# Jimmy2027/MoPoE-MIMIC

Hardware: AMD Instinct MI355X
Metric: samples/sec (higher is better)
Workload: dtype f32

## Files before the change

### include/mopoe_hip.h

```cpp
#ifndef MOPOE_HIP_H
#define MOPOE_HIP_H

#include <stddef.h>
#include <stdint.h>

#ifdef __cplusplus
extern "C" {
#endif

#define MOPOE_ABI_VERSION 20

#define MOPOE_OK 0
#define MOPOE_ERR_ARG (-1)
#define MOPOE_ERR_LAUNCH (-2)
#define MOPOE_ERR_DEVICE (-3)

int mopoe_abi_version(void);
const char* mopoe_last_error(void);

typedef struct {
  int32_t N;
  int32_t Hs, Ws;
  int32_t Hb, Wb;
  int32_t Cin, Cout;
  int32_t kh, kw;
  int32_t sh, sw;
  int32_t ph, pw;
  int32_t transposed;
} mopoe_conv_geom;

typedef struct {
  const double* sums;
  const float* gamma;
  const float* beta;
  const float* rmean;
  const float* rvar;
  double inv_count;
  float eps;
  int32_t C;
  int32_t mode;
} mopoe_bn_ref;

typedef struct {
  const float* mask;
  int32_t kind;
  int32_t rows_per_sample;
} mopoe_mask_ref;

size_t mopoe_conv_workspace_bytes(void);

typedef struct {
  int32_t tile;
  int32_t split;
} mopoe_conv_plan;

int mopoe_conv_fwd(const float* x, const float* wp, const float* bias, float* y,
                   const mopoe_conv_geom* g, const mopoe_bn_ref* bn_in, const mopoe_mask_ref* mask,
                   double* out_stats, const mopoe_conv_plan* plan, void* workspace, size_t workspace_bytes,
                   void* stream);

typedef struct {
  const void* s;
  mopoe_bn_ref bn;
  float a, b;
} mopoe_mix_ref;
int mopoe_conv_fwd_mix(const float* x, const float* wp, const float* bias, float* y, const mopoe_conv_geom* g,
                       const mopoe_bn_ref* bn_in, const mopoe_mask_ref* mask, const mopoe_mix_ref* mix,
                       double* out_stats, const mopoe_conv_plan* plan, void* workspace, size_t workspace_bytes,
                       void* stream);

int mopoe_conv_dgrad(const float* dy, const float* wp, float* dx, const mopoe_conv_geom* g,
                     const mopoe_bn_ref* relu_bn, const float* xin, double* bwd_sums,
                     const mopoe_conv_plan* plan, void* workspace, size_t workspace_bytes, void* stream);

int mopoe_conv_wgrad(const float* x, const float* dy, float* dwp, const mopoe_conv_geom* g,
                     const mopoe_bn_ref* bn_in, int32_t dwp_is_zero, const mopoe_conv_plan* plan, void* stream);

int mopoe_block_out_fwd(const float* s, const float* m, float* out, int64_t rows, int32_t C,
                        const mopoe_bn_ref* bn_s, float a, float b, double* out_stats, void* stream);

int mopoe_bn_relu_apply(const float* x, float* out, int64_t rows, int32_t C, const mopoe_bn_ref* bn, void* stream);

int mopoe_bn_bwd_reduce(const float* g, const float* s, int64_t rows, int32_t C,
                        const mopoe_bn_ref* bn_s, double* sums, void* stream);

int mopoe_block_out_bwd(const float* g, const float* s, float* dm, float* ds, int64_t rows, int32_t C,
                        const mopoe_bn_ref* bn_s, const double* sums, const mopoe_mask_ref* mask,
                        float a, float b, float* dgamma, float* dbeta, float* colsum_dm,
                        float* colsum_ds, void* stream);

int mopoe_bn_bwd_apply(const float* dy, const float* x, const float* add, float* dx, int64_t rows,
                       int32_t C, const mopoe_bn_ref* bn, const double* sums,
                       const mopoe_mask_ref* mask, float* dgamma, float* dbeta, float* colsum_dx,
                       const float* next_s, const mopoe_bn_ref* next_bn, double* next_sums, void* stream);

typedef struct {
  const double* sums;
  float* rmean;
  float* rvar;
  int32_t C;
  int32_t count;
} mopoe_bn_running_desc;
int mopoe_bn_running_update(const mopoe_bn_running_desc* desc, int32_t n, float momentum, void* stream);

int mopoe_colsum(const float* x, float* out, int64_t rows, int32_t C, int32_t out_is_zero, void* stream);

int mopoe_latent_fwd(const float* const mu_in[3], const float* const lv_in[3], const float* eps,
                     int32_t B, int32_t D, const int32_t* row_start, const float* w, float norm,
                     float* mus, float* lvs, float* joint_mu, float* joint_lv, float* z, float* klds,
                     float* joint_div, double* kl_ws, void* stream);

int mopoe_latent_bwd(const float* const mu_in[3], const float* const lv_in[3], const float* eps,
                     int32_t B, int32_t D, const int32_t* row_start, const float* w, float norm,
                     const float* g_mus, const float* g_lvs, const float* g_joint_mu,
                     const float* g_joint_lv, const float* g_z, const float* g_klds,
                     const float* g_joint_div, float* const d_mu_in[3], float* const d_lv_in[3],
                     void* stream);

#define MOPOE_LATENT_MOE 0
#define MOPOE_LATENT_JSD 1
int mopoe_latent_mixture_fwd(int32_t method, const float* const mu_in[3], const float* const lv_in[3],
                             const float* eps, int32_t B, int32_t D, const int32_t* member_row_start,
                             const int32_t* comp_row_start, const float* w, float norm, float* sub_mu,
                             float* sub_lv, float* comp_mu, float* comp_lv, float* joint_mu, float* joint_lv,
                             float* z, float* klds, float* individual_divs, float* joint_div, float* pd_mu,
                             float* pd_lv, double* ws, void* stream);

int mopoe_latent_mixture_bwd(int32_t method, const float* const mu_in[3], const float* const lv_in[3],
                             const float* eps, int32_t B, int32_t D, const int32_t* member_row_start,
                             const int32_t* comp_row_start, const float* w, float norm, const float* g_sub_mu,
                             const float* g_sub_lv, const float* g_comp_mu, const float* g_comp_lv,
                             const float* g_joint_mu, const float* g_joint_lv, const float* g_z,
                             const float* g_klds, const float* g_individual_divs, const float* g_joint_div,
                             const float* g_pd_mu, const float* g_pd_lv, float* const d_mu_in[3],
                             float* const d_lv_in[3], void* stream);

// ... 13 lines not shown
int mopoe_dense_nll_fwd(const float* logp, const float* target, int64_t n, float norm, float* out, double* ws,
                        void* stream);
int mopoe_dense_nll_bwd(const float* target, const float* g, int64_t n, float norm, float* dlogp, void* stream);

int mopoe_laplace_logprob_rows(const float* x_hat, const float* x, int64_t rows, int64_t per_row,
                               int64_t target_rows, float scale, float* out, void* stream);
int mopoe_token_logprob_rows(const float* logp, const float* ids, int64_t rows, int32_t L, int32_t V,
                             int64_t target_rows, float* out, void* stream);
int mopoe_token_softmax_grad(const float* logp, const float* ids, const float* g, int64_t rows, int32_t V, float norm,
                             void* dx, int32_t dx_is_bf16, void* stream);
int mopoe_block_front_stats_bf16(const uint16_t* x, const uint16_t* w1, const float* bias, int64_t rows, int32_t C,
                                 const mopoe_bn_ref* bn1, const mopoe_mask_ref* mask1, double* stats_d1, void* stream);
int mopoe_block_front_apply_bf16(const uint16_t* x, const uint16_t* w1, const float* bias, uint16_t* a2, int64_t rows, int32_t C,
                                 const mopoe_bn_ref* bn1, const mopoe_bn_ref* bn2, const mopoe_mask_ref* mask1, void* stream);
int mopoe_block_front_bwd_bf16(const uint16_t* x, const uint16_t* dh2, const uint16_t* w1, const float* bias, uint16_t* dh1,
                               int64_t rows, int32_t C, const mopoe_bn_ref* bn1, const mopoe_bn_ref* bn2,
                               const mopoe_mask_ref* mask1, const double* sums2, double* sums1, float* dw1, float* dbias,
                               float* dgamma2, float* dbeta2, void* stream);
int mopoe_block_front_stats(const float* x, const float* w1, const float* bias, int64_t rows, int32_t C,
                            const mopoe_bn_ref* bn1, const mopoe_mask_ref* mask1, double* stats_d1, void* stream);
int mopoe_block_front_apply(const float* x, const float* w1, const float* bias, float* a2, int64_t rows, int32_t C,
                            const mopoe_bn_ref* bn1, const mopoe_bn_ref* bn2, const mopoe_mask_ref* mask1, void* stream);
int mopoe_block_front_bwd(const float* x, const float* dh2, const float* w1, const float* bias, float* dh1, int64_t rows, int32_t C,
                          const mopoe_bn_ref* bn1, const mopoe_bn_ref* bn2, const mopoe_mask_ref* mask1, const double* sums2,
                          double* sums1, float* dw1, float* dbias, float* dgamma2, float* dbeta2, void* stream);
int mopoe_lse_rows(const void* logits, int32_t is_bf16, int64_t rows, int32_t V, float* lse, void* stream);
int mopoe_token_nll_logits_fwd(const void* logits, int32_t is_bf16, const float* lse, const float* ids, int64_t rows, int32_t V,
                               float norm, float* out, double* ws, void* stream);
int mopoe_token_softmax_grad_logits(const void* logits, int32_t is_bf16, const float* lse, const float* ids, const float* g,
                                    int64_t rows, int32_t V, float norm, void* dx, void* stream);
int mopoe_dense_logprob_rows(const float* logp, const float* target, int64_t rows, int64_t per_row,
                             int64_t target_rows, float* out, void* stream);

int mopoe_embedding_fwd(const float* ids, const float* table, float* out, int64_t rows, int32_t V,
                        int32_t D, void* stream);
int mopoe_embedding_bwd(const float* ids, const float* gout, float* dtable, int64_t rows, int32_t V,
                        int32_t D, int32_t padding_idx, void* stream);


int mopoe_conv_fwd_bf16(const uint16_t* x, const uint16_t* wp, const float* bias, void* y, int32_t y_is_f32,
                        const mopoe_conv_geom* g, const mopoe_bn_ref* bn_in, const mopoe_mask_ref* mask,
                        double* out_stats, const mopoe_conv_plan* plan, void* workspace, size_t workspace_bytes,
                        void* stream);
int mopoe_conv_fwd_mix_bf16(const uint16_t* x, const uint16_t* wp, const float* bias, uint16_t* y,
                            const mopoe_conv_geom* g, const mopoe_bn_ref* bn_in, const mopoe_mask_ref* mask,
                            const mopoe_mix_ref* mix, double* out_stats, const mopoe_conv_plan* plan, void* workspace,
                            size_t workspace_bytes, void* stream);
int mopoe_conv_dgrad_bf16(const uint16_t* dy, const uint16_t* wp, void* dx, int32_t dx_is_f32, const mopoe_conv_geom* g,
                          const mopoe_bn_ref* relu_bn, const uint16_t* xin, double* bwd_sums,
                          const mopoe_conv_plan* plan, void* workspace, size_t workspace_bytes, void* stream);
int mopoe_conv_wgrad_bf16(const uint16_t* x, const uint16_t* dy, float* dwp, const mopoe_conv_geom* g,
                          const mopoe_bn_ref* bn_in, int32_t dwp_is_zero, const mopoe_conv_plan* plan, void* stream);
int mopoe_edge_expand_bf16(const float* scal, const float* w, uint16_t* out, const mopoe_conv_geom* g, int32_t C,
                           double* stats, void* stream);
int mopoe_edge_wgrad_bf16(const uint16_t* vec, const float* scal, float* dw, const mopoe_conv_geom* g, int32_t C,
                          int32_t dw_is_zero, void* stream);
int mopoe_edge_reduce_bf16(const uint16_t* x, const float* w, const float* bias, float* out, const mopoe_conv_geom* g,
                           int32_t C, void* stream);
int mopoe_bn_relu_apply_bf16(const uint16_t* x, uint16_t* out, int64_t rows, int32_t C, const mopoe_bn_ref* bn, void* stream);
int mopoe_block_out_fwd_bf16(const uint16_t* s, const uint16_t* m, uint16_t* out, int64_t rows, int32_t C,
                             const mopoe_bn_ref* bn_s, float a, float b, double* out_stats, void* stream);
int mopoe_bn_bwd_reduce_bf16(const uint16_t* g, const uint16_t* s, int64_t rows, int32_t C, const mopoe_bn_ref* bn_s,
                             double* sums, void* stream);
int mopoe_block_out_bwd_bf16(const uint16_t* g, const uint16_t* s, uint16_t* dm, uint16_t* ds, int64_t rows, int32_t C,
                             const mopoe_bn_ref* bn_s, const double* sums, const mopoe_mask_ref* mask, float a, float b,
                             float* dgamma, float* dbeta, float* colsum_dm, float* colsum_ds, void* stream);
int mopoe_bn_bwd_apply_bf16(const uint16_t* dy, const uint16_t* x, const uint16_t* add, uint16_t* dx, int64_t rows,
                            int32_t C, const mopoe_bn_ref* bn, const double* sums, const mopoe_mask_ref* mask,
                            float* dgamma, float* dbeta, float* colsum_dx, const uint16_t* next_s,
                            const mopoe_bn_ref* next_bn, double* next_sums, void* stream);
int mopoe_colsum_bf16(const uint16_t* x, float* out, int64_t rows, int32_t C, int32_t out_is_zero, void* stream);
int mopoe_logsoftmax_bwd_bf16out(const float* dy, const float* y, uint16_t* dx, int64_t rows, int32_t V, void* stream);
int mopoe_embedding_fwd_bf16(const float* ids, const float* table, uint16_t* out, int64_t rows, int32_t V, int32_t D,
                             void* stream);
int mopoe_embedding_bwd_bf16(const float* ids, const uint16_t* gout, float* dtable, int64_t rows, int32_t V, int32_t D,
                             int32_t padding_idx, void* stream);

typedef struct {
  float* p;
  const float* g;
  float* m;
  float* v;
  uint16_t* p16;
  int64_t n;
} mopoe_adam_seg;
int mopoe_adam_step(const mopoe_adam_seg* segs, int32_t nseg, float* step, const float* lr_dev, double lr, double beta1,
                    double beta2, double eps, float* coef, void* stream);

#define MOPOE_PROF_KINDS 144
int mopoe_prof_enable(int32_t on);
int mopoe_prof_stamp(uint64_t* slot, void* stream);
int mopoe_prof_collect(int64_t* launches, double* total_ms, double* total_flops, double* total_bytes );

#ifdef __cplusplus
}
#endif
#endif
```

### mopoe-mimic_amd/csrc/adam.hip

```cpp
#include "common.hpp"

namespace mopoe {

constexpr int ADAM_SEGS_PER_LAUNCH = 64;
constexpr int ADAM_CHUNK = 4096;
constexpr int ADAM_THREADS = 256;

struct AdamPack {
  mopoe_adam_seg seg[ADAM_SEGS_PER_LAUNCH];
  int chunk_start[ADAM_SEGS_PER_LAUNCH];
};

__global__ void adam_prep_kernel(float* step, const float* lr_dev, double lr_host, double beta1, double beta2, float* coef) {
  if (threadIdx.x != 0 || blockIdx.x != 0) return;
  const float s = step[0] + 1.f;
  step[0] = s;
  const double lr = lr_dev ? (double)lr_dev[0] : lr_host;
  const float bc1 = (float)(1.0 - pow(beta1, (double)s));
  const float bc2s = (float)sqrt(1.0 - pow(beta2, (double)s));
  coef[0] = (float)(lr / (double)bc1);
  coef[1] = bc2s;
}

struct AdamHyper {
  double beta1, beta2, eps;
  float step_size, bc2_sqrt;
};

__device__ __forceinline__ void adam_one(float& p, float g, float& m, float& v, const AdamHyper& h) {
  m = (float)(h.beta1 * (double)m + (1.0 - h.beta1) * (double)g);
  v = (float)(h.beta2 * (double)v + (1.0 - h.beta2) * (double)g * (double)g);
  const float denom = (float)((double)(sqrtf(v) / h.bc2_sqrt) + h.eps);
  p -= h.step_size * m / denom;
}

__global__ __launch_bounds__(ADAM_THREADS) void adam_kernel(const AdamPack pack, int nseg, const float* __restrict__ coef,
                                                            double beta1, double beta2, double eps) {
  const int tid = threadIdx.x, lane = tid & 63;
  const int b = (int)blockIdx.x;
  static_assert(ADAM_SEGS_PER_LAUNCH == 64, "one prefix entry per lane");
  const unsigned long long le = __ballot(pack.chunk_start[lane] <= b);
  const int si = __builtin_amdgcn_readfirstlane(__popcll(le) - 1);
  if (si < 0 || si >= nseg) return;
  const mopoe_adam_seg s = pack.seg[si];
  const long base = (long)(b - pack.chunk_start[si]) * ADAM_CHUNK;
  AdamHyper h;
  h.beta1 = beta1; h.beta2 = beta2; h.eps = eps;
  h.step_size = coef[0]; h.bc2_sqrt = coef[1];

  const bool vec = ((((uintptr_t)s.p | (uintptr_t)s.g | (uintptr_t)s.m | (uintptr_t)s.v) & 15) == 0) &&
                   (s.p16 == nullptr || (((uintptr_t)s.p16) & 7) == 0);
  if (vec) {
    float4 p[4], g[4], m[4], v[4];
    bool ok[4];
#pragma unroll
    for (int i = 0; i < 4; ++i) {
      const long e = base + (long)(i * ADAM_THREADS + tid) * 4;
      ok[i] = e + 3 < s.n;
      if (ok[i]) {
        g[i] = *reinterpret_cast<const float4*>(s.g + e);
        p[i] = *reinterpret_cast<const float4*>(s.p + e);
        m[i] = *reinterpret_cast<const float4*>(s.m + e);
        v[i] = *reinterpret_cast<const float4*>(s.v + e);
      }
    }
#pragma unroll
    for (int i = 0; i < 4; ++i) {
      if (!ok[i]) continue;
      const long e = base + (long)(i * ADAM_THREADS + tid) * 4;
      adam_one(p[i].x, g[i].x, m[i].x, v[i].x, h);
      adam_one(p[i].y, g[i].y, m[i].y, v[i].y, h);
      adam_one(p[i].z, g[i].z, m[i].z, v[i].z, h);
      adam_one(p[i].w, g[i].w, m[i].w, v[i].w, h);
      *reinterpret_cast<float4*>(s.p + e) = p[i];
      *reinterpret_cast<float4*>(s.m + e) = m[i];
      *reinterpret_cast<float4*>(s.v + e) = v[i];
      if (s.p16) {
        uint2 o;
        o.x = pack_bf16(p[i].x, p[i].y);
        o.y = pack_bf16(p[i].z, p[i].w);
        *reinterpret_cast<uint2*>(s.p16 + e) = o;
      }
    }
    const long tail = s.n & ~3L;
    if (tid == 0 && tail >= base && tail < base + ADAM_CHUNK) {
      for (long e = tail; e < s.n; ++e) {
        float pp = s.p[e], mm = s.m[e], vv = s.v[e];
        adam_one(pp, s.g[e], mm, vv, h);
        s.p[e] = pp; s.m[e] = mm; s.v[e] = vv;
        if (s.p16) s.p16[e] = f32_to_bf16(pp);
      }
    }
  } else {
    for (int i = tid; i < ADAM_CHUNK; i += ADAM_THREADS) {
      const long e = base + i;
      if (e >= s.n) break;
      float pp = s.p[e], mm = s.m[e], vv = s.v[e];
      adam_one(pp, s.g[e], mm, vv, h);
      s.p[e] = pp; s.m[e] = mm; s.v[e] = vv;
      if (s.p16) s.p16[e] = f32_to_bf16(pp);
    }
  }
}

}

using namespace mopoe;

extern "C" int mopoe_adam_step(const mopoe_adam_seg* segs, int32_t nseg, float* step, const float* lr_dev, double lr,
                               double beta1, double beta2, double eps, float* coef, void* stream) {
  if ((!segs && nseg != 0) || nseg < 0 || !coef) { set_error("adam_step: bad arguments"); return MOPOE_ERR_ARG; }
  hipStream_t st = (hipStream_t)stream;
  if (step) {
    hipLaunchKernelGGL(adam_prep_kernel, dim3(1), dim3(64), 0, st, step, lr_dev, lr, beta1, beta2, coef);
    if (int rc = check_launch("adam_prep")) return rc;
  }
  int32_t i = 0;
  while (i < nseg) {
    AdamPack pack;
    int n = 0;
    long blocks = 0;
    for (; i < nseg && n < ADAM_SEGS_PER_LAUNCH; ++i) {
      const mopoe_adam_seg& s = segs[i];
      if (!s.g || s.n == 0) continue;
      if (!s.p || !s.m || !s.v || s.n < 0) { set_error("adam_step: record %d is incomplete", (int)i); return MOPOE_ERR_ARG; }
      const long nb = (s.n + ADAM_CHUNK - 1) / ADAM_CHUNK;
      if (nb > 0x7fffffffL) { set_error("adam_step: record %d has more than 2^43 elements", (int)i); return MOPOE_ERR_ARG; }
      if (blocks + nb > 0x7fffffffL) break;
      pack.seg[n] = s;
      pack.chunk_start[n] = (int)blocks;
      blocks += nb;
      ++n;
    }
    for (int k = n; k < ADAM_SEGS_PER_LAUNCH; ++k) { pack.seg[k] = mopoe_adam_seg{}; pack.chunk_start[k] = 0x7fffffff; }
    if (n == 0) continue;
    hipLaunchKernelGGL(adam_kernel, dim3((unsigned)blocks), dim3(ADAM_THREADS), 0, st, pack, n, coef, beta1, beta2, eps);
    if (int rc = check_launch("adam_step")) return rc;
  }
  return MOPOE_OK;
}
```

### mopoe-mimic_amd/csrc/conv_gemm.hip

```cpp
#include "gemm_common.hpp"

namespace mopoe {

constexpr int BK = 16;
#ifndef TILE_N64_REMAINDER
#define TILE_N64_REMAINDER 64
#endif
#ifndef SPLIT_BLOCKS
#define SPLIT_BLOCKS 256
#endif
#ifndef SPLIT_TARGET
#define SPLIT_TARGET 512
#endif
#ifndef GEMM_8WAVES
#define GEMM_8WAVES 1
#endif
#ifndef PERSIST_BLOCKS
#define PERSIST_BLOCKS 2048
#endif
#ifndef GEMM_MIN_WAVES
#define GEMM_MIN_WAVES 3
#endif
#ifndef GEMM_BK_BIG
#define GEMM_BK_BIG 16
#endif
#ifndef GEMM_LDS_PAD
#define GEMM_LDS_PAD 4
#endif
constexpr int LDS_PAD = GEMM_LDS_PAD;

struct GemmArgs {
  const float* X;
  const float* W;
  float* Y;
  const float* bias;
  int N, Hx, Wx, Hy, Wy, Ck, Cn, Cin_w, Cout_w;
  int kh, kw, sh, sw, ph, pw;
  int form, w_nk;
  int Hq, Wq;
  long rows_per_phase;
  int vecA, vecB;
  mopoe_bn_ref bn_in;
  mopoe_mask_ref mask;
  double* out_stats;
  mopoe_bn_ref relu_bn;
  const float* xin;
  double* bwd_sums;
  unsigned x_bytes, w_bytes;
  int nsplit;
  float* partial;
  int* counters;
  long rows_total;
  int mix;
  float mix_a, mix_b;
  int xcd_remap;
};

__device__ __forceinline__ float epi_round(const GemmArgs&, float x) { return x; }
struct EpiXinRaw { float4 lo, hi; };
constexpr bool EPI_PREFETCH_XIN = false;
__device__ __forceinline__ EpiXinRaw epi_xin_ld(const GemmArgs& a, long yrow, int ncol, bool ok_hi) {
  const float* p = a.xin + yrow * a.Cn + ncol;
  EpiXinRaw r;
  r.lo = *reinterpret_cast<const float4*>(p);
  r.hi = ok_hi ? *reinterpret_cast<const float4*>(p + 4) : make_float4(0.f, 0.f, 0.f, 0.f);
  return r;
}
__device__ __forceinline__ void epi_xin_unpack(const EpiXinRaw& r, float (&xi)[8]) {
  xi[0] = r.lo.x; xi[1] = r.lo.y; xi[2] = r.lo.z; xi[3] = r.lo.w; xi[4] = r.hi.x; xi[5] = r.hi.y; xi[6] = r.hi.z; xi[7] = r.hi.w;
}
__device__ __forceinline__ void epi_store8(const GemmArgs& a, long yrow, int ncol, bool ok_hi, const float (&v)[8]) {
  float* dst = a.Y + yrow * a.Cn + ncol;
  *reinterpret_cast<float4*>(dst) = make_float4(v[0], v[1], v[2], v[3]);
  if (ok_hi) *reinterpret_cast<float4*>(dst + 4) = make_float4(v[4], v[5], v[6], v[7]);
}


__device__ __forceinline__ float4 bld4(__amdgpu_buffer_rsrc_t srd, unsigned byte_off) {
  const u32x4 v = __builtin_amdgcn_raw_buffer_load_b128(srd, byte_off, 0, 0);
  return make_float4(__uint_as_float(v.x), __uint_as_float(v.y), __uint_as_float(v.z), __uint_as_float(v.w));
}

__device__ __forceinline__ float4 bld4s(__amdgpu_buffer_rsrc_t srd, unsigned byte_off, unsigned s_off) {
  const u32x4 v = __builtin_amdgcn_raw_buffer_load_b128(srd, byte_off, s_off, 0);
  return make_float4(__uint_as_float(v.x), __uint_as_float(v.y), __uint_as_float(v.z), __uint_as_float(v.w));
}

__device__ __forceinline__ float4 ld4(const float* p, int nvalid, bool vec) {
  float4 v = make_float4(0.f, 0.f, 0.f, 0.f);
  if (nvalid >= 4 && vec) {
    v = *reinterpret_cast<const float4*>(p);
  } else {
    if (nvalid > 0) v.x = p[0];
    if (nvalid > 1) v.y = p[1];
    if (nvalid > 2) v.z = p[2];
    if (nvalid > 3) v.w = p[3];
  }
  return v;
}

template <int BM, int BN, int WGM, int WGN, int GBK, bool VEC, int SPEC = 0>
__global__ __launch_bounds__(64 * WGM * WGN, (WGM * WGN == 4 ? GEMM_MIN_WAVES : ((BM / WGM) * (BN / WGN) > 64 * 32 ? 2 : 4)))
void gather_gemm_kernel(const GemmArgs a) {
  static_assert(SPEC == 0 || VEC, "specialised loops exist for the vector path only");
  constexpr int NT = 64 * WGM * WGN;
  static_assert(WGM * WGN == 4 || WGM * WGN == 8, "4 or 8 waves per block");
  constexpr int WM = BM / WGM, WN = BN / WGN;
  constexpr int TI = WM / 32, TJ = WN / 32;
  constexpr int A_LD = BM + LDS_PAD, B_LD = BN + LDS_PAD;
  constexpr int KQ = GBK / 4;
  constexpr int RPP = NT / KQ;
  constexpr int A_PER_THR = BM / RPP;
  static_assert(BM % RPP == 0, "A tile rows must be a multiple of the rows covered per pass");
  constexpr int B_PER_THR_NK = (BN + RPP - 1) / RPP;
  constexpr int N4 = BN / 4;
  constexpr int B_PER_THR_KN = (GBK * N4 + NT - 1) / NT;
  constexpr int B_PER_THR = B_PER_THR_NK > B_PER_THR_KN ? B_PER_THR_NK : B_PER_THR_KN;

  constexpr int STG_LD = WN + 4;
  constexpr int A_FLOATS = 2 * GBK * A_LD, B_FLOATS = 2 * GBK * B_LD;
  constexpr int STG_FLOATS = VEC ? (NT / 64) * 32 * STG_LD : 0;
  constexpr int SMEM_FLOATS = (A_FLOATS + B_FLOATS) > STG_FLOATS ? (A_FLOATS + B_FLOATS) : STG_FLOATS;
  __shared__ __attribute__((aligned(16))) float smem[SMEM_FLOATS];
  __shared__ __attribute__((aligned(16))) float bnS[MAX_BN_C];
  __shared__ __attribute__((aligned(16))) float bnT[MAX_BN_C];
  __shared__ __attribute__((aligned(16))) float epi[5][VEC ? BN : 4];
  __shared__ int s_ticket;
  float* const As0 = smem;
  float* const Bs0 = smem + A_FLOATS;
#define AS_(buf, k, r) As0[((buf) * GBK + (k)) * A_LD + (r)]
#define BS_(buf, k, r) Bs0[((buf) * GBK + (k)) * B_LD + (r)]

  const int tid = threadIdx.x;
  const int lane = tid & 63, wave = tid >> 6;
  const int wm = wave / WGN, wn = wave % WGN;
  unsigned lbx = blockIdx.x, lby = blockIdx.y, lbz = blockIdx.z;
  if (a.xcd_remap) {
    const unsigned inner = gridDim.y * gridDim.z;
// ... 780 lines not shown
__global__ __launch_bounds__(256) void splitk_epilogue_kernel(const GemmArgs a) {
  __shared__ float cs[2][4][64];
  const int tx = threadIdx.x & 63, ty = threadIdx.x >> 6;
  const int n = blockIdx.x * 64 + tx;
  const bool nok = n < a.Cn;
  const bool do_relu_bn = a.relu_bn.mode != 0;
  const float bias = (nok && a.bias) ? a.bias[n] : 0.f;
  BnC rb = {0.f, 0.f, 0.f, 0.f};
  if (nok && do_relu_bn) rb = bn_coef(a.relu_bn, n);
  const long stride = a.rows_total * (long)a.Cn;
  float s1 = 0.f, s2 = 0.f;
  if (nok) {
    for (long row = (long)blockIdx.y * 4 + ty; row < a.rows_total; row += (long)gridDim.y * 4) {
      const float* p = a.partial + row * a.Cn + n;
      float acc8[8] = {0.f, 0.f, 0.f, 0.f, 0.f, 0.f, 0.f, 0.f};
      int s = 0;
      for (; s + 8 <= a.nsplit; s += 8) {
#pragma unroll
        for (int u = 0; u < 8; ++u) acc8[u] += p[(long)(s + u) * stride];
      }
      for (; s < a.nsplit; ++s) acc8[s & 7] += p[(long)s * stride];
      float x = bias + (((acc8[0] + acc8[1]) + (acc8[2] + acc8[3])) + ((acc8[4] + acc8[5]) + (acc8[6] + acc8[7])));
      if (a.mask.kind != 0) x *= mask_at(a.mask, row, n, a.Cn);
      if (do_relu_bn) {
        const float xi = a.xin[row * a.Cn + n];
        x = (fmaf(xi, rb.scale, rb.shift) > 0.f) ? x : 0.f;
        s1 += x;
        s2 += x * ((xi - rb.mean) * rb.rstd);
      } else {
        s1 += x;
        s2 += x * x;
      }
      a.Y[row * a.Cn + n] = x;
    }
  }
  double* sums = do_relu_bn ? a.bwd_sums : a.out_stats;
  if (sums) {
    cs[0][ty][tx] = s1;
    cs[1][ty][tx] = s2;
    __syncthreads();
    if (ty == 0 && nok) {
      atomic_add_f64(sums + n, (double)((cs[0][0][tx] + cs[0][1][tx]) + (cs[0][2][tx] + cs[0][3][tx])));
      atomic_add_f64(sums + a.Cn + n, (double)((cs[1][0][tx] + cs[1][1][tx]) + (cs[1][2][tx] + cs[1][3][tx])));
    }
  }
}


#include "gemm_glds_common.inc"
#include "conv_gemm_glds.inc"
#include "conv_gemm_glds_parity.inc"


static int launch_gather(const float* X, const float* W, const float* bias, float* Y, const mopoe_conv_geom* g,
                         int dest_on_small, int Ck, int Cn, int w_nk, const mopoe_bn_ref* bn_in,
                         const mopoe_mask_ref* mask, double* out_stats, const mopoe_bn_ref* relu_bn,
                         const float* xin, double* bwd_sums, const mopoe_conv_plan* plan, void* ws, size_t ws_bytes,
                         hipStream_t stream, const mopoe_mix_ref* mix = nullptr) {
  int* counters = nullptr;
  if (ws && ws_bytes > WS_COUNTER_BYTES) { counters = (int*)ws; ws = (char*)ws + WS_COUNTER_BYTES; ws_bytes -= WS_COUNTER_BYTES; }
  else { ws = nullptr; ws_bytes = 0; }
  GemmArgs a;
  a.X = X; a.W = W; a.Y = Y; a.bias = bias;
  a.N = g->N; a.Ck = Ck; a.Cn = Cn; a.Cin_w = g->Cin; a.Cout_w = g->Cout;
  a.kh = g->kh; a.kw = g->kw; a.sh = g->sh; a.sw = g->sw; a.ph = g->ph; a.pw = g->pw;
  a.w_nk = w_nk;
  int nphase;
  if (dest_on_small) {
    a.form = 0; a.Hx = g->Hb; a.Wx = g->Wb; a.Hy = g->Hs; a.Wy = g->Ws; a.Hq = g->Hs; a.Wq = g->Ws; nphase = 1;
  } else {
    a.form = 1; a.Hx = g->Hs; a.Wx = g->Ws; a.Hy = g->Hb; a.Wy = g->Wb; a.Hq = g->Hb / g->sh; a.Wq = g->Wb / g->sw;
    nphase = g->sh * g->sw;
  }
  a.rows_per_phase = (long)g->N * a.Hq * a.Wq;
  a.rows_total = (long)g->N * a.Hy * a.Wy;
  a.vecA = (Ck % 4 == 0) && aligned16(X);
  a.vecB = (g->Cout % 4 == 0) && aligned16(W);
  const size_t xb = (size_t)g->N * a.Hx * a.Wx * Ck * sizeof(float);
  const size_t wb = (size_t)g->kh * g->kw * g->Cin * g->Cout * sizeof(float);
  const bool vec = a.vecA && a.vecB && xb < (1ull << 31) && wb < (1ull << 31) && Cn % 4 == 0 && aligned16(Y) &&
                   (!xin || aligned16(xin)) && (!mask || mask->kind == 0 || aligned16(mask->mask));
  a.x_bytes = (unsigned)std::min<size_t>(xb, 0x7fffffffu);
  a.w_bytes = (unsigned)std::min<size_t>(wb, 0x7fffffffu);
  mopoe_bn_ref none = {};
  mopoe_mask_ref nomask = {nullptr, 0, 1};
  a.bn_in = bn_in ? *bn_in : none;
  a.mask = mask ? *mask : nomask;
  a.out_stats = out_stats;
  a.relu_bn = relu_bn ? *relu_bn : none;
  a.xin = xin; a.bwd_sums = bwd_sums;
  a.mix = 0; a.mix_a = a.mix_b = 0.f;
  static const bool xcd_remap_g = !getenv("MOPOE_NO_XCD_REMAP");
  a.xcd_remap = xcd_remap_g ? 1 : 0;
  if (mix) {
    if (!mix->s || mix->bn.mode == 0 || relu_bn || xin) { set_error("conv_fwd_mix: needs s and its BatchNorm"); return MOPOE_ERR_ARG; }
    if (!vec || !aligned16(mix->s)) { set_error("conv_fwd_mix: channel counts must be multiples of 4 and tensors 16-byte aligned"); return MOPOE_ERR_ARG; }
    a.mix = 1; a.mix_a = mix->a; a.mix_b = mix->b;
    a.relu_bn = mix->bn; a.xin = (const float*)mix->s;
  }
  a.nsplit = 1; a.partial = nullptr; a.counters = nullptr;
  static const bool dbg_nostats = getenv("MOPOE_DEBUG_NOSTATS") != nullptr;
  if (dbg_nostats) { a.out_stats = nullptr; a.bwd_sums = nullptr; }
  if (a.bn_in.mode != 0 && (a.bn_in.C != Ck || Ck > MAX_BN_C)) { set_error("bn_in channel mismatch (%d vs %d)", a.bn_in.C, Ck); return MOPOE_ERR_ARG; }
  if (a.relu_bn.mode != 0 && (a.relu_bn.C != Cn || !a.xin)) { set_error("relu_bn needs xin and C == %d", Cn); return MOPOE_ERR_ARG; }
  if (a.mask.kind != 0 && !a.mask.mask) { set_error("mask pointer missing"); return MOPOE_ERR_ARG; }
  if (a.mask.kind == 1 && a.mask.rows_per_sample != a.Hy * a.Wy) { set_error("channel mask: rows_per_sample must be Hout*Wout"); return MOPOE_ERR_ARG; }
  if (a.rows_total >= (1L << 31) || (long)g->N * a.Hx * a.Wx >= (1L << 31)) { set_error("conv: more than 2^31 rows"); return MOPOE_ERR_ARG; }

  int cfg;
  bool emu = false;
  if (Cn > 64) cfg = (a.rows_per_phase > 64 || Cn >= 256) ? 0 : 2;
  else cfg = a.rows_per_phase >= 256L * 64 ? 1 : 2;
#ifdef TILE_N64_REMAINDER
  if (cfg == 0 && (Cn % 128) == 64 && a.rows_per_phase >= 256L * TILE_N64_REMAINDER) cfg = 1;
#endif
  if (plan && plan->tile >= 0) {
    if (plan->tile > 19) { set_error("conv plan: tile %d (see mopoe_conv_plan in mopoe_hip.h: 0..19)", plan->tile); return MOPOE_ERR_ARG; }
    cfg = plan->tile;
    if (cfg >= 16) {
      if (a.bn_in.mode != 0) { set_error("conv plan: tile %d (split-bf16 products) has no BN-on-load form", cfg); return MOPOE_ERR_ARG; }
      emu = true;
      cfg -= 4;
    }
    if (cfg >= 12 && (!vec || Ck % 32 != 0 || (a.bn_in.mode != 0 && cfg == 13))) {
      set_error("conv plan: tile %d (LDS-DMA family) needs the vector path, K channels %% 32 == 0 (Ck = %d) and, with BN on load, tile 12, 14 or 15", cfg, Ck);
      return MOPOE_ERR_ARG;
    }
    if (cfg >= 3 && !vec) cfg = cfg == 3 ? 0 : 2;
    if ((cfg == 5 || cfg == 6) && Ck % 32 != 0) cfg -= 3;
    if (cfg >= 8 && cfg < 12 && (!vec || Ck % 8 != 0 || a.mix)) cfg = (cfg == 8) ? 0 : (cfg == 9 ? 1 : (cfg == 10 ? 2 : 4));
  }
  static const int TILE_BM[16] = {128, 256, 64, 256, 128, 64, 128, 128, 128, 256, 64, 128, 128, 128, 64, 256};
  static const int TILE_BN[16] = {128, 64, 64, 128, 64, 64, 64, 128, 128, 64, 64, 64, 128, 64, 64, 128};
  const int bm = TILE_BM[cfg], bn = TILE_BN[cfg];
  const long nMt = ceil_div(a.rows_per_phase, bm);
  const int nNt = ceil_div(Cn, bn);
  const int gbk = (cfg == 5 || cfg == 6 || cfg >= 12) ? 32 : (cfg >= 8 ? 8 : 16);
  const int nkc = ceil_div(Ck, gbk);
  const int iters = (dest_on_small ? g->kh * g->kw : std::max(1, (g->kh / g->sh) * (g->kw / g->sw))) * nkc;
  const long blocks = nMt * nNt * nphase;
  const size_t per = (size_t)a.rows_total * Cn * sizeof(float);
  if (plan && plan->split > 0) {
    long ns = std::min<long>(plan->split, iters);
    if (ns >= 2 && (!ws || (size_t)ns * per > ws_bytes)) {
      set_error("conv plan: split %ld needs %zu workspace bytes (have %zu)", ns, (size_t)ns * per, ws ? ws_bytes : (size_t)0);
      return MOPOE_ERR_ARG;
    }
    if (ns >= 2) { a.nsplit = (int)ns; a.partial = (float*)ws; }
  } else if (ws && blocks < SPLIT_BLOCKS && iters * gbk >= 256) {
    long ns = std::min<long>((SPLIT_TARGET + blocks - 1) / blocks, (long)iters * gbk / 128);
    if ((size_t)ns * per > ws_bytes) ns = (long)(ws_bytes / per);
    if (ns >= 2) { a.nsplit = (int)ns; a.partial = (float*)ws; }
  }
  const bool in_kernel_reduce = vec && (cfg < 8 || cfg >= 12);
  if (a.partial && in_kernel_reduce) {
    if (blocks > (long)(WS_COUNTER_BYTES / sizeof(int))) { set_error("conv: split reduction over %ld output tiles (at most %zu)", blocks, WS_COUNTER_BYTES / sizeof(int)); return MOPOE_ERR_ARG; }
    a.counters = counters;
  }
  const long persist = cfg >= 12 ? (cfg == 15 ? 256 : 512)
                                 : (cfg >= 8 ? 4096 : ((cfg == 2 || cfg >= 4) ? PERSIST_BLOCKS * 3 / 2 : PERSIST_BLOCKS));
  long gx = std::min<long>(nMt, std::max<long>(1, persist / ((long)nNt * nphase * a.nsplit)));
  double taps_eff = dest_on_small ? (double)g->kh * g->kw : (double)g->kh * g->kw / ((double)g->sh * g->sw);
  const double flops = 2.0 * (double)g->N * a.Hy * a.Wy * (double)Cn * (double)Ck * taps_eff;
  {
    const int spec = (vec && Ck % gbk == 0) ? (w_nk ? 3 : (a.bn_in.mode != 0 ? 2 : 1)) : 0;
    const double abytes = ((double)g->N * a.Hx * a.Wx * Ck + (double)a.rows_total * Cn) * sizeof(float);
    ProfScope prof(stream, flops, emu ? PROF_F32_GLDS_EMU + (cfg - 12) * 2 + (spec == 3 ? 1 : 0)
                                      : cfg >= 12 ? PROF_F32_GLDS + (cfg - 12) * 3 + (spec - 1)
                                            : (cfg >= 8 ? PROF_DIRECT + (cfg - 8) * 4 + spec
                                                        : (vec ? PROF_GATHER_VEC + cfg * 4 + spec : PROF_GATHER_SCALAR + cfg)), abytes);
    dim3 grid((unsigned)gx, nNt, nphase * a.nsplit);
#define MOPOE_LAUNCH_TILE(BM_, BN_, WM_, WN_, BK_, THREADS_)                                                                    \
  do {                                                                                                                          \
    if (spec == 1) hipLaunchKernelGGL((gather_gemm_kernel<BM_, BN_, WM_, WN_, BK_, true, 1>), grid, dim3(THREADS_), 0, stream, a);      \
    else if (spec == 2) hipLaunchKernelGGL((gather_gemm_kernel<BM_, BN_, WM_, WN_, BK_, true, 2>), grid, dim3(THREADS_), 0, stream, a); \
    else if (spec == 3) hipLaunchKernelGGL((gather_gemm_kernel<BM_, BN_, WM_, WN_, BK_, true, 3>), grid, dim3(THREADS_), 0, stream, a); \
    else hipLaunchKernelGGL((gather_gemm_kernel<BM_, BN_, WM_, WN_, 16, true, 0>), grid, dim3(THREADS_), 0, stream, a);                \
  } while (0)
#define MOPOE_LAUNCH_DIRECT(WM_, WN_, TI_, TJ_)                                                                                   \
  do {                                                                                                                          \
    if (spec == 1) hipLaunchKernelGGL((direct_gemm_kernel<WM_, WN_, TI_, TJ_, 1>), grid, dim3(64 * WM_ * WN_), 0, stream, a);      \
    else if (spec == 2) hipLaunchKernelGGL((direct_gemm_kernel<WM_, WN_, TI_, TJ_, 2>), grid, dim3(64 * WM_ * WN_), 0, stream, a); \
    else hipLaunchKernelGGL((direct_gemm_kernel<WM_, WN_, TI_, TJ_, 3>), grid, dim3(64 * WM_ * WN_), 0, stream, a);                \
  } while (0)
#define MOPOE_LAUNCH_GLDS(BM_, BN_, WM_, WN_, ST_)                                                                                       \
  do {                                                                                                                                \
    if (spec == 1) hipLaunchKernelGGL((gather_gemm_f32_glds_kernel<BM_, BN_, WM_, WN_, 1, ST_>), grid, dim3(64 * WM_ * WN_), 0, stream, a); \
    else hipLaunchKernelGGL((gather_gemm_f32_glds_kernel<BM_, BN_, WM_, WN_, 3, ST_>), grid, dim3(64 * WM_ * WN_), 0, stream, a);          \
  } while (0)
#define MOPOE_LAUNCH_GLDS_EMU(BM_, BN_, WM_, WN_, ST_)                                                                                   \
  do {                                                                                                                                \
    if (spec == 1) hipLaunchKernelGGL((gather_gemm_f32_glds_kernel<BM_, BN_, WM_, WN_, 1, ST_, 1>), grid, dim3(64 * WM_ * WN_), 0, stream, a); \
    else hipLaunchKernelGGL((gather_gemm_f32_glds_kernel<BM_, BN_, WM_, WN_, 3, ST_, 1>), grid, dim3(64 * WM_ * WN_), 0, stream, a);          \
  } while (0)
    if (emu) {
      if (cfg == 12) MOPOE_LAUNCH_GLDS_EMU(128, 128, 2, 2, 2);
      else if (cfg == 13) MOPOE_LAUNCH_GLDS_EMU(128, 64, 2, 2, 3);
      else if (cfg == 14) MOPOE_LAUNCH_GLDS_EMU(64, 64, 2, 2, 4);
      else MOPOE_LAUNCH_GLDS_EMU(256, 128, 4, 2, 3);
    }
#undef MOPOE_LAUNCH_GLDS_EMU
    else if (cfg >= 12) {
      if (spec == 2) {
        if (cfg == 12) hipLaunchKernelGGL((gather_gemm_f32_glds_kernel<128, 128, 2, 2, 2, 2>), grid, dim3(256), 0, stream, a);
        else if (cfg == 14) hipLaunchKernelGGL((gather_gemm_f32_glds_kernel<64, 64, 2, 2, 2, 4>), grid, dim3(256), 0, stream, a);
        else hipLaunchKernelGGL((gather_gemm_f32_glds_kernel<256, 128, 4, 2, 2, 2>), grid, dim3(512), 0, stream, a);
      }
      else if (cfg == 12) MOPOE_LAUNCH_GLDS(128, 128, 2, 2, 2);
      else if (cfg == 13) MOPOE_LAUNCH_GLDS(128, 64, 2, 2, 3);
      else if (cfg == 14) MOPOE_LAUNCH_GLDS(64, 64, 2, 2, 4);
      else MOPOE_LAUNCH_GLDS(256, 128, 4, 2, 2);
    }
#undef MOPOE_LAUNCH_GLDS
    else if (cfg == 8) MOPOE_LAUNCH_DIRECT(2, 2, 2, 2);
    else if (cfg == 9) MOPOE_LAUNCH_DIRECT(4, 1, 2, 2);
    else if (cfg == 10) MOPOE_LAUNCH_DIRECT(2, 2, 1, 1);
    else if (cfg == 11) MOPOE_LAUNCH_DIRECT(2, 1, 2, 2);
    else if (vec) {
      if (cfg == 0) MOPOE_LAUNCH_TILE(128, 128, 2, 4, 16, 512);
      else if (cfg == 1) MOPOE_LAUNCH_TILE(256, 64, 4, 2, 16, 512);
      else if (cfg == 3) MOPOE_LAUNCH_TILE(256, 128, 4, 2, 16, 512);
      else if (cfg == 4) MOPOE_LAUNCH_TILE(128, 64, 2, 2, 16, 256);
      else if (cfg == 5) MOPOE_LAUNCH_TILE(64, 64, 2, 2, 32, 256);
      else if (cfg == 6) MOPOE_LAUNCH_TILE(128, 64, 2, 2, 32, 256);
      else if (cfg == 7) MOPOE_LAUNCH_TILE(128, 128, 2, 2, 16, 256);
      else MOPOE_LAUNCH_TILE(64, 64, 2, 2, 16, 256);
    } else {
      if (cfg == 0) hipLaunchKernelGGL((gather_gemm_kernel<128, 128, 2, 2, GEMM_BK_BIG, false>), grid, dim3(256), 0, stream, a);
      else if (cfg == 1) hipLaunchKernelGGL((gather_gemm_kernel<256, 64, 4, 1, 16, false>), grid, dim3(256), 0, stream, a);
      else hipLaunchKernelGGL((gather_gemm_kernel<64, 64, 2, 2, 16, false>), grid, dim3(256), 0, stream, a);
    }
#undef MOPOE_LAUNCH_TILE
#undef MOPOE_LAUNCH_DIRECT
    if (int rc = check_launch("gather_gemm")) return rc;
    if (a.partial && !in_kernel_reduce) {
      dim3 eg(ceil_div(Cn, 64), std::min<long>(ceil_div(a.rows_total, 4), EPI_MAX_BLOCKS_Y));
      hipLaunchKernelGGL(splitk_epilogue_kernel, eg, dim3(256), 0, stream, a);
      if (int rc = check_launch("splitk_epilogue")) return rc;
    }
  }
  return MOPOE_OK;
}

}

using namespace mopoe;

extern "C" size_t mopoe_conv_workspace_bytes(void) { return WS_RECOMMENDED; }

extern "C" int mopoe_conv_fwd(const float* x, const float* wp, const float* bias, float* y, const mopoe_conv_geom* g,
                              const mopoe_bn_ref* bn_in, const mopoe_mask_ref* mask, double* out_stats,
                              const mopoe_conv_plan* plan, void* workspace, size_t workspace_bytes, void* stream) {
  if (int rc = validate_geom(g)) return rc;
  if (!x || !wp || !y) { set_error("conv_fwd: null pointer"); return MOPOE_ERR_ARG; }
  const bool plain = (!bn_in || bn_in->mode == 0) && (!mask || mask->kind == 0);
  if (plain && !g->transposed && g->Cin == 1 && !bias && edge_supported(g, g->Cout, {wp, y}))
    return edge_expand(x, wp, y, g, g->Cout, out_stats, (hipStream_t)stream);
  if (plain && g->transposed && g->Cout == 1 && !out_stats && edge_supported(g, g->Cin, {x, wp}))
    return edge_reduce(x, wp, bias, y, g, g->Cin, (hipStream_t)stream);
  return launch_gather(x, wp, bias, y, g, g->transposed ? 0 : 1, g->Cin, g->Cout, 0, bn_in, mask, out_stats,
                       nullptr, nullptr, nullptr, plan, workspace, workspace_bytes, (hipStream_t)stream);
}

extern "C" int mopoe_conv_fwd_mix(const float* x, const float* wp, const float* bias, float* y, const mopoe_conv_geom* g,
                                  const mopoe_bn_ref* bn_in, const mopoe_mask_ref* mask, const mopoe_mix_ref* mix,
                                  double* out_stats, const mopoe_conv_plan* plan, void* workspace, size_t workspace_bytes,
                                  void* stream) {
  if (int rc = validate_geom(g)) return rc;
  if (!x || !wp || !y || !mix) { set_error("conv_fwd_mix: null pointer"); return MOPOE_ERR_ARG; }
  return launch_gather(x, wp, bias, y, g, g->transposed ? 0 : 1, g->Cin, g->Cout, 0, bn_in, mask, out_stats,
                       nullptr, nullptr, nullptr, plan, workspace, workspace_bytes, (hipStream_t)stream, mix);
}

extern "C" int mopoe_conv_dgrad(const float* dy, const float* wp, float* dx, const mopoe_conv_geom* g,
                                const mopoe_bn_ref* relu_bn, const float* xin, double* bwd_sums,
                                const mopoe_conv_plan* plan, void* workspace, size_t workspace_bytes, void* stream) {
  if (int rc = validate_geom(g)) return rc;
  if (!dy || !wp || !dx) { set_error("conv_dgrad: null pointer"); return MOPOE_ERR_ARG; }
  if (g->transposed && g->Cout == 1 && (!relu_bn || relu_bn->mode == 0) && edge_supported(g, g->Cin, {wp, dx}))
    return edge_expand(dy, wp, dx, g, g->Cin, nullptr, (hipStream_t)stream);
  return launch_gather(dy, wp, nullptr, dx, g, g->transposed ? 1 : 0, g->Cout, g->Cin, 1, nullptr, nullptr,
                       nullptr, relu_bn, xin, bwd_sums, plan, workspace, workspace_bytes, (hipStream_t)stream);
}

// ... 130 lines not shown
```

### mopoe-mimic_amd/csrc/conv_gemm_bf16_glds.inc

```
#include "gemm_glds_common.inc"

#ifdef MOPOE_DBG_NO_DMA
#define MOPOE_DBG_DMA(x) do { } while (0)
#else
#define MOPOE_DBG_DMA(x) x
#endif
#ifdef MOPOE_DBG_NO_MFMA
#define MOPOE_DBG_MFMA(x) do { } while (0)
#else
#define MOPOE_DBG_MFMA(x) x
#endif

template <int OFF>
__device__ __forceinline__ void lds_frag_b128(bf16x8& r, unsigned addr) {
  static_assert(OFF >= 0 && OFF < 65536, "ds offset field");
  MOPOE_DEVICE_ASM("ds_read_b128 %0, %1 offset:%2" : "=v"(r) : "v"(addr), "n"(OFF) : "memory");
}
template <int OFF>
__device__ __forceinline__ void lds_frag_tr64(s16x4& r, unsigned addr) {
  static_assert(OFF >= 0 && OFF < 65536, "ds offset field");
  MOPOE_DEVICE_ASM("ds_read_b64_tr_b16 %0, %1 offset:%2" : "=v"(r) : "v"(addr), "n"(OFF) : "memory");
}
template <int TI, int TJ>
__device__ __forceinline__ void fence_frags(bf16x8 (&fa)[TI], bf16x8 (&fb)[TJ]) {
  static_assert(TI <= 2 && TJ <= 2, "operand list written for wave tiles of at most 64 x 64");
  if constexpr (TI == 2 && TJ == 2) MOPOE_DEVICE_ASM("s_waitcnt lgkmcnt(0)" : "+v"(fa[0]), "+v"(fa[1]), "+v"(fb[0]), "+v"(fb[1]) :: "memory");
  else if constexpr (TI == 1 && TJ == 2) MOPOE_DEVICE_ASM("s_waitcnt lgkmcnt(0)" : "+v"(fa[0]), "+v"(fb[0]), "+v"(fb[1]) :: "memory");
  else if constexpr (TI == 2 && TJ == 1) MOPOE_DEVICE_ASM("s_waitcnt lgkmcnt(0)" : "+v"(fa[0]), "+v"(fa[1]), "+v"(fb[0]) :: "memory");
  else MOPOE_DEVICE_ASM("s_waitcnt lgkmcnt(0)" : "+v"(fa[0]), "+v"(fb[0]) :: "memory");
  __builtin_amdgcn_sched_barrier(0);
}
template <int TI, int TJ>
__device__ __forceinline__ void fence_frags_tr(bf16x8 (&fa)[TI], s16x4 (&lo)[TJ], s16x4 (&hi)[TJ]) {
  static_assert(TI <= 2 && TJ <= 2, "operand list written for wave tiles of at most 64 x 64");
  if constexpr (TI == 2 && TJ == 2)
    MOPOE_DEVICE_ASM("s_waitcnt lgkmcnt(0)" : "+v"(fa[0]), "+v"(fa[1]), "+v"(lo[0]), "+v"(lo[1]), "+v"(hi[0]), "+v"(hi[1]) :: "memory");
  else if constexpr (TI == 1 && TJ == 2)
    MOPOE_DEVICE_ASM("s_waitcnt lgkmcnt(0)" : "+v"(fa[0]), "+v"(lo[0]), "+v"(lo[1]), "+v"(hi[0]), "+v"(hi[1]) :: "memory");
  else if constexpr (TI == 2 && TJ == 1)
    MOPOE_DEVICE_ASM("s_waitcnt lgkmcnt(0)" : "+v"(fa[0]), "+v"(fa[1]), "+v"(lo[0]), "+v"(hi[0]) :: "memory");
  else MOPOE_DEVICE_ASM("s_waitcnt lgkmcnt(0)" : "+v"(fa[0]), "+v"(lo[0]), "+v"(hi[0]) :: "memory");
  __builtin_amdgcn_sched_barrier(0);
}

template <int BM, int BN, int WGM, int WGN, int SPEC, int NSTAGE>
__global__ __launch_bounds__(64 * WGM * WGN, 2) void gather_gemm_bf16_glds_kernel(const GemmArgsH a) {
  constexpr int NT = 64 * WGM * WGN, NW = NT / 64;
  constexpr int WM = BM / WGM, WN = BN / WGN;
  constexpr int TI = WM / 32, TJ = WN / 32;
  static_assert(TI >= 1 && TJ >= 1 && WM % 32 == 0 && WN % 32 == 0, "wave tile is made of 32x32 MFMA tiles");
  static_assert(SPEC >= 1 && SPEC <= 3, "SPEC");
  static_assert(NSTAGE >= 2 && NSTAGE <= 4, "two to four LDS buffers");
  constexpr int R = (SPEC == 2 && NSTAGE == 4) ? 4 : 1;
  static_assert(NW % 2 == 0, "the swizzled chunk of a lane is the same for all its rows only with an even wave count");
  constexpr bool xform = SPEC == 2;
  static_assert(BN == 64 || BN == 128, "swizzle of the K-strided image is written for 128- and 256-byte rows");
  constexpr bool w_nk = SPEC == 3;
  constexpr int BKG = 64;
  constexpr int A_BYTES = BM * 128;
  constexpr int B_ROWB = w_nk ? 128 : BN * 2;
  constexpr int B_BYTES = BN * 128;
  constexpr int STAGE_BYTES = A_BYTES + B_BYTES;
  constexpr int A_INSTR = A_BYTES / (NT * 16), B_INSTR = B_BYTES / (NT * 16);
  static_assert(A_BYTES % (NT * 16) == 0 && B_BYTES % (NT * 16) == 0 && A_INSTR >= 1 && B_INSTR >= 1, "whole 1-KB pieces per wave");
  constexpr int LPS = A_INSTR + B_INSTR;
  constexpr int B_LPR = B_ROWB / 16;
  constexpr int B_RPP = 64 / B_LPR;

  constexpr int STG_LD = WN + 4;
  constexpr int STG_BYTES = NW * 32 * STG_LD * 4;
  constexpr int TILE_BYTES = NSTAGE * STAGE_BYTES > STG_BYTES ? NSTAGE * STAGE_BYTES : STG_BYTES;
  constexpr int OFF_EPI = TILE_BYTES, OFF_TICKET = OFF_EPI + 5 * BN * 4, OFF_BN = OFF_TICKET + 16;
  __shared__ __attribute__((aligned(1024))) unsigned char smem[OFF_BN + (xform ? 2 * MAX_BN_C * 4 : 0)];
  float (*const epi)[BN] = reinterpret_cast<float (*)[BN]>(smem + OFF_EPI);
  int& s_ticket = *reinterpret_cast<int*>(smem + OFF_TICKET);
  float* const bnS = reinterpret_cast<float*>(smem + OFF_BN);
  float* const bnT = bnS + MAX_BN_C;
  bool was_last = false;

  const int tid = threadIdx.x;
  const int lane = tid & 63, wave = __builtin_amdgcn_readfirstlane(tid >> 6);
  const int wm = wave / WGN, wn = wave % WGN;
  unsigned lbx = blockIdx.x, lby = blockIdx.y, lbz = blockIdx.z;
  if (a.xcd_remap) {
    const unsigned inner = gridDim.y * gridDim.z;
    const unsigned sw = xcd_swizzle(blockIdx.x + gridDim.x * (blockIdx.y + gridDim.y * blockIdx.z), gridDim.x * inner);
    lbx = sw / inner;
    const unsigned rem = sw - lbx * inner;
    lby = rem % gridDim.y;
    lbz = rem / gridDim.y;
  }
  const int n0 = lby * BN;
  const int phase = lbz / a.nsplit;
  const int split = lbz - phase * a.nsplit;

  const TapWalk tw = tap_walk(a, phase);
  const int ntx = tw.ntx, ky0 = tw.ky0, kx0 = tw.kx0, kstep_y = tw.kstep_y, kstep_x = tw.kstep_x;
  const int dsgn = tw.dsgn, cy = tw.cy, cx = tw.cx, phy = tw.phy, phx = tw.phx;
  const int nkc = a.Ck / BKG;
  const int total_all = tw.nty * ntx * nkc;
  const __amdgpu_buffer_rsrc_t srdX = __builtin_amdgcn_make_buffer_rsrc((void*)a.X, 0, (int)a.x_bytes, 0x00020000);
  const __amdgpu_buffer_rsrc_t srdW = __builtin_amdgcn_make_buffer_rsrc((void*)a.W, 0, (int)a.w_bytes, 0x00020000);
  const int per_split = (total_all + a.nsplit - 1) / a.nsplit;
  const int it_beg = split * per_split;
  const int it_end = it_beg + per_split < total_all ? it_beg + per_split : total_all;
  const int total = it_end > it_beg ? it_end - it_beg : 0;

  const int l31 = lane & 31, lhi = lane >> 5;
  const bool do_relu_bn = a.relu_bn.mode != 0 && !a.mix;
  const int hw = a.Hq * a.Wq;

  if (xform) {
    for (int c = tid; c < a.Ck; c += NT) {
      const BnC k = bn_coef(a.bn_in, c);
      bnS[c] = k.scale;
      bnT[c] = k.shift;
    }
  }
  for (int c = tid; c < BN; c += NT) {
    const int n = n0 + c;
    BnC k = BnC{0.f, 0.f, 0.f, 0.f};
    if (n < a.Cn && (do_relu_bn || a.mix)) k = bn_coef(a.relu_bn, n);
    if (a.mix) { k.scale *= a.mix_a; k.shift *= a.mix_a; }
    epi[0][c] = k.mean; epi[1][c] = k.rstd; epi[2][c] = k.scale; epi[3][c] = k.shift;
    epi[4][c] = (n < a.Cn && a.bias) ? a.bias[n] : 0.f;
  }
  __syncthreads();
  constexpr int E_LPR = WN / 8, E_RPP = 64 / E_LPR, E_NPASS = 32 / E_RPP;
  const int c8 = lane % E_LPR, rsub = lane / E_LPR;
  const int ecol = wn * WN + c8 * 8;
  const int ncol = n0 + ecol;
  const bool ok_lo = ncol < a.Cn, ok_hi = ok_lo;
  float s1[8], s2[8];
#pragma unroll
  for (int e = 0; e < 8; ++e) s1[e] = s2[e] = 0.f;
  float* const stg = reinterpret_cast<float*>(smem) + wave * 32 * STG_LD;
  const unsigned lds_base = (unsigned)(uintptr_t)((lds_void_t*)smem);

  unsigned voffB[B_INSTR];
#pragma unroll
  for (int i = 0; i < B_INSTR; ++i) {
    const int pc = i * NW + wave;
    if (w_nk) {
      const int r = 8 * pc + (lane >> 3);
      const int cq = (lane & 7) ^ ((r >> 1) & 7);
      const int n = n0 + r;
      voffB[i] = n < a.Cn ? ((unsigned)n * (unsigned)a.Cout_w + (unsigned)cq * 8u) * 2u : OOB;
    } else {
      const int k = B_RPP * pc + lane / B_LPR;
      const int g = BN == 128 ? (k & 3) : ((k >> 1) & 1);
      const int cq = (lane % B_LPR) ^ (g << 2);
      const int n = n0 + cq * 8;
      voffB[i] = n < a.Cn ? ((unsigned)k * (unsigned)a.Cout_w + (unsigned)n) * 2u : OOB;
    }
  }
  unsigned aoff[TI][4];
#pragma unroll
  for (int i = 0; i < TI; ++i) {
    const int r = wm * WM + i * 32 + l31;
#pragma unroll
    for (int s = 0; s < 4; ++s) aoff[i][s] = (unsigned)r * 128u + (unsigned)(((2 * s + lhi) ^ ((r >> 1) & 7)) * 16);
  }
  unsigned boff[TJ][w_nk ? 4 : 1];
#pragma unroll
  for (int j = 0; j < TJ; ++j) {
    if (w_nk) {
      const int r = wn * WN + j * 32 + l31;
#pragma unroll
      for (int s = 0; s < (w_nk ? 4 : 1); ++s)
        boff[j][s] = (unsigned)A_BYTES + (unsigned)r * 128u + (unsigned)(((2 * s + lhi) ^ ((r >> 1) & 7)) * 16);
    } else {
      const int i16 = lane & 15, g16 = (lane >> 4) & 1;
      const int k = lhi * 8 + (i16 >> 2);
      const int colb = (wn * WN + j * 32 + g16 * 16 + (i16 & 3) * 4) * 2;
      const int g = BN == 128 ? (k & 3) : ((k >> 1) & 1);
      boff[j][0] = (unsigned)A_BYTES + (unsigned)k * (unsigned)B_ROWB + (unsigned)((((colb >> 4) ^ (g << 2)) << 4) | (colb & 15));
    }
  }

  const long nMt = (a.rows_per_phase + BM - 1) / BM;
  for (long mt = lbx; mt < nMt; mt += gridDim.x) {
    const long m0 = mt * BM;

    int ry0[A_INSTR], rx0[A_INSTR], rbase[A_INSTR];
    unsigned cqA[A_INSTR];
    bool rvalid[A_INSTR];
#pragma unroll
    for (int i = 0; i < A_INSTR; ++i) {
      const int r = 8 * (i * NW + wave) + (lane >> 3);
      cqA[i] = (unsigned)(((lane & 7) ^ ((r >> 1) & 7)) * 16);
      const long m = m0 + r;
      rvalid[i] = m < a.rows_per_phase;
      const unsigned mm = rvalid[i] ? (unsigned)m : 0u;
      const int n = (int)(mm / (unsigned)hw);
      const int rem = (int)(mm - (unsigned)n * (unsigned)hw);
      const int qy = rem / a.Wq, qx = rem - qy * a.Wq;
      if (a.form == 0) { ry0[i] = qy * a.sh - a.ph; rx0[i] = qx * a.sw - a.pw; }
      else             { ry0[i] = qy + cy;          rx0[i] = qx + cx; }
      rbase[i] = (n * a.Hx + ry0[i]) * a.Wx + rx0[i];
    }

    int ld_tap = it_beg / nkc;
    int ld_kc = (it_beg - ld_tap * nkc) * BKG;
    bool tap_dirty = true;
    unsigned offA[A_INSTR], offW = 0;

    u32x4 ra[R][xform ? A_INSTR : 1];
    unsigned pend_ok[R][xform ? A_INSTR : 1];
    int kch_set[R];
    unsigned sB_set[R];

    auto issue = [&](auto bufc) {
      constexpr int buf = decltype(bufc)::value;
      if (tap_dirty) {
        const int jy = ld_tap / ntx, jx = ld_tap - jy * ntx;
        const int wtap = (ky0 + kstep_y * jy) * a.kw + (kx0 + kstep_x * jx);
        const int tapoff = dsgn * (jy * a.Wx + jx);
#pragma unroll
        for (int i = 0; i < A_INSTR; ++i) {
          const int iy = ry0[i] + dsgn * jy, ix = rx0[i] + dsgn * jx;
          const bool ok = rvalid[i] & ((unsigned)iy < (unsigned)a.Hx) & ((unsigned)ix < (unsigned)a.Wx);
          offA[i] = ok ? (unsigned)(rbase[i] + tapoff) * (unsigned)a.ldx * 2u + cqA[i] : OOB;

        }
        offW = (unsigned)wtap * (unsigned)a.Cin_w * (unsigned)a.Cout_w * 2u;
        tap_dirty = false;
      }
      const unsigned sA = (unsigned)ld_kc * 2u;
      const unsigned sB = offW + (w_nk ? (unsigned)ld_kc * 2u : (unsigned)ld_kc * (unsigned)a.Cout_w * 2u);
      unsigned char* const stage = smem + buf * STAGE_BYTES;
      if constexpr (xform) {
        constexpr int set = buf;
        kch_set[set] = ld_kc + (int)(cqA[0] >> 1);
#pragma unroll
        for (int i = 0; i < A_INSTR; ++i) { ra[set][i] = __builtin_amdgcn_raw_buffer_load_b128(srdX, offA[i], sA, 0); pend_ok[set][i] = offA[i] == OOB ? 0u : 0xffffffffu; }
        sB_set[set] = sB;
      } else {
#pragma unroll
        for (int i = 0; i < A_INSTR; ++i)
          MOPOE_DBG_DMA(lds_dma16(srdX, stage + (i * NW + wave) * 1024, offA[i], sA));
      }
      if constexpr (!xform) {
#pragma unroll
        for (int i = 0; i < B_INSTR; ++i)
          MOPOE_DBG_DMA(lds_dma16(srdW, stage + A_BYTES + (i * NW + wave) * 1024, voffB[i], sB));
      }
      ld_kc += BKG;
      if (ld_kc >= a.Ck) { ld_kc = 0; ++ld_tap; tap_dirty = true; }
    };
    auto commit = [&](auto bufc, auto setc) {
      constexpr int buf = decltype(bufc)::value, set = xform ? decltype(setc)::value : 0;
      unsigned char* const stage = smem + buf * STAGE_BYTES;
      if constexpr (xform) {
        u32x4 c0, c1, c2, c3;
        lds_load_coef4(c0, c1, c2, c3, lds_base + (unsigned)OFF_BN + (unsigned)kch_set[set] * 4u,
                       lds_base + (unsigned)OFF_BN + (unsigned)(MAX_BN_C + kch_set[set]) * 4u);
        const float4 psc0 = __builtin_bit_cast(float4, c0), psc1 = __builtin_bit_cast(float4, c1);
        const float4 psh0 = __builtin_bit_cast(float4, c2), psh1 = __builtin_bit_cast(float4, c3);
#pragma unroll
// ... 657 lines not shown
```

### mopoe-mimic_amd/csrc/conv_gemm_glds.inc

```
typedef float f32x4v __attribute__((ext_vector_type(4)));

template <int OFF>
__device__ __forceinline__ void lds_frag_f4(f32x4v& r, unsigned addr) {
  static_assert(OFF >= 0 && OFF < 65536, "ds offset field");
  MOPOE_DEVICE_ASM("ds_read_b128 %0, %1 offset:%2" : "=v"(r) : "v"(addr), "n"(OFF) : "memory");
}
template <int OFF>
__device__ __forceinline__ void lds_frag_f1(float& r, unsigned addr) {
  static_assert(OFF >= 0 && OFF < 65536, "ds offset field");
  MOPOE_DEVICE_ASM("ds_read_b32 %0, %1 offset:%2" : "=v"(r) : "v"(addr), "n"(OFF) : "memory");
}

typedef __bf16 e_bf16x2 __attribute__((ext_vector_type(2)));
typedef __bf16 e_bf16x8 __attribute__((ext_vector_type(8)));
typedef float e_f32x2 __attribute__((ext_vector_type(2)));
struct Split3 { u32x4 h, m, l; };

__device__ __forceinline__ void split3_pair(float a0, float a1, unsigned& h, unsigned& m, unsigned& l) {
#if defined(MOPOE_DBG_EMU_NOSPLIT)
  h = __float_as_uint(a0); m = __float_as_uint(a1); l = h;
  return;
#endif
  const e_f32x2 a = {a0, a1};
  h = __builtin_bit_cast(unsigned, __builtin_convertvector(a, e_bf16x2));
  float r0 = 0.f, r1 = 0.f, q0 = 0.f, q1 = 0.f;
  MOPOE_DEVICE_ASM_PURE("v_sub_f32 %0, %1, %2" : "=v"(r0) : "v"(a0), "v"(h << 16));
  MOPOE_DEVICE_ASM_PURE("v_sub_f32 %0, %1, %2" : "=v"(r1) : "v"(a1), "v"(h & 0xffff0000u));
  const e_f32x2 r = {r0, r1};
  m = __builtin_bit_cast(unsigned, __builtin_convertvector(r, e_bf16x2));
  MOPOE_DEVICE_ASM_PURE("v_sub_f32 %0, %1, %2" : "=v"(q0) : "v"(r0), "v"(m << 16));
  MOPOE_DEVICE_ASM_PURE("v_sub_f32 %0, %1, %2" : "=v"(q1) : "v"(r1), "v"(m & 0xffff0000u));
  const e_f32x2 r2 = {q0, q1};
  l = __builtin_bit_cast(unsigned, __builtin_convertvector(r2, e_bf16x2));
}
__device__ __forceinline__ void split3_first(float a0, float a1, unsigned& h, float& r0, float& r1) {
  const e_f32x2 a = {a0, a1};
  h = __builtin_bit_cast(unsigned, __builtin_convertvector(a, e_bf16x2));
  MOPOE_DEVICE_ASM_PURE("v_sub_f32 %0, %1, %2" : "=v"(r0) : "v"(a0), "v"(h << 16));
  MOPOE_DEVICE_ASM_PURE("v_sub_f32 %0, %1, %2" : "=v"(r1) : "v"(a1), "v"(h & 0xffff0000u));
}
__device__ __forceinline__ void split3_second(float r0, float r1, unsigned& m, unsigned& l) {
  const e_f32x2 r = {r0, r1};
  m = __builtin_bit_cast(unsigned, __builtin_convertvector(r, e_bf16x2));
  float q0 = 0.f, q1 = 0.f;
  MOPOE_DEVICE_ASM_PURE("v_sub_f32 %0, %1, %2" : "=v"(q0) : "v"(r0), "v"(m << 16));
  MOPOE_DEVICE_ASM_PURE("v_sub_f32 %0, %1, %2" : "=v"(q1) : "v"(r1), "v"(m & 0xffff0000u));
  const e_f32x2 q = {q0, q1};
  l = __builtin_bit_cast(unsigned, __builtin_convertvector(q, e_bf16x2));
}
__device__ __forceinline__ Split3 split3(const float (&v0)[4], const float (&v1)[4]) {
  unsigned h[4], m[4], l[4];
  split3_pair(v0[0], v0[1], h[0], m[0], l[0]);
  split3_pair(v0[2], v0[3], h[1], m[1], l[1]);
  split3_pair(v1[0], v1[1], h[2], m[2], l[2]);
  split3_pair(v1[2], v1[3], h[3], m[3], l[3]);
  Split3 s;
  s.h = u32x4{h[0], h[1], h[2], h[3]};
  s.m = u32x4{m[0], m[1], m[2], m[3]};
  s.l = u32x4{l[0], l[1], l[2], l[3]};
  return s;
}
__device__ __forceinline__ Split3 split3(const f32x4v& v0, const f32x4v& v1) {
  const float a[4] = {v0[0], v0[1], v0[2], v0[3]}, b[4] = {v1[0], v1[1], v1[2], v1[3]};
  return split3(a, b);
}
__device__ __forceinline__ f32x16 mfma_bf16(const u32x4& a, const u32x4& b, const f32x16& c) {
  return __builtin_amdgcn_mfma_f32_32x32x16_bf16(__builtin_bit_cast(e_bf16x8, a), __builtin_bit_cast(e_bf16x8, b), c, 0, 0, 0);
}
__device__ __forceinline__ void mfma_split6(f32x16& acc, const Split3& a, const Split3& b) {
  acc = mfma_bf16(a.h, b.l, acc);
  acc = mfma_bf16(a.l, b.h, acc);
  acc = mfma_bf16(a.m, b.m, acc);
  acc = mfma_bf16(a.h, b.m, acc);
  acc = mfma_bf16(a.m, b.h, acc);
  acc = mfma_bf16(a.h, b.h, acc);
}
template <int TERM>
__device__ __forceinline__ void mfma_split_term(f32x16& acc, const Split3& a, const Split3& b) {
#if defined(MOPOE_DBG_EMU_NOMFMA)
  MOPOE_DEVICE_ASM("" :: "v"(a.h), "v"(a.m), "v"(a.l), "v"(b.h), "v"(b.m), "v"(b.l));
#else
  const u32x4& x = TERM == 1 ? a.l : ((TERM == 2 || TERM == 4) ? a.m : a.h);
  const u32x4& y = TERM == 0 ? b.l : ((TERM == 2 || TERM == 3) ? b.m : b.h);
  acc = mfma_bf16(x, y, acc);
#endif
}
template <typename T>
__device__ __forceinline__ void pin_reg(T& r) { MOPOE_DEVICE_ASM("" : "+v"(r)); }

template <int BM, int BN, int WGM, int WGN, int SPEC, int NSTAGE, int EMU = 0>
__global__ __launch_bounds__(64 * WGM * WGN, 2) void gather_gemm_f32_glds_kernel(const GemmArgs a) {
  constexpr int NT = 64 * WGM * WGN, NW = NT / 64;
  constexpr int WM = BM / WGM, WN = BN / WGN;
  constexpr int TI = WM / 32, TJ = WN / 32;
  static_assert(TI >= 1 && TJ >= 1 && TI <= 2 && TJ <= 2 && WM % 32 == 0 && WN % 32 == 0, "wave tile: one to four 32x32 MFMA tiles");
  static_assert(SPEC >= 1 && SPEC <= 3, "SPEC");
  static_assert(NSTAGE >= 2 && NSTAGE <= 4 && (SPEC != 2 || NSTAGE == 2 || NSTAGE == 4), "two to four LDS buffers (two or four with BN on load)");
  constexpr int R = NSTAGE == 4 ? 2 : 1;
  static_assert(NW % 2 == 0, "the swizzled chunk of a lane is the same for all its rows only with an even wave count");
  static_assert(BN == 64 || BN == 128, "column tiles of 64 or 128");
  constexpr bool xform = SPEC == 2;
  constexpr bool w_nk = SPEC == 3;
  constexpr int BKG = 32;
  constexpr int A_BYTES = BM * 128;
  constexpr int B_ROWB = w_nk ? 128 : BN * 4;
  constexpr int B_BYTES = BN * 128;
  constexpr int STAGE_BYTES = A_BYTES + B_BYTES;
  constexpr int A_INSTR = A_BYTES / (NT * 16), B_INSTR = B_BYTES / (NT * 16);
  static_assert(A_BYTES % (NT * 16) == 0 && B_BYTES % (NT * 16) == 0 && A_INSTR >= 1 && B_INSTR >= 1, "whole 1-KB pieces per wave");
  constexpr int LPS = A_INSTR + B_INSTR;
  constexpr int B_LPR = B_ROWB / 16, B_RPP = 64 / B_LPR;

  constexpr int STG_LD = WN + 4;
  constexpr int STG_BYTES = NW * 32 * STG_LD * 4;
  constexpr int TILE_BYTES = NSTAGE * STAGE_BYTES > STG_BYTES ? NSTAGE * STAGE_BYTES : STG_BYTES;
  constexpr int OFF_EPI = TILE_BYTES, OFF_TICKET = OFF_EPI + 5 * BN * 4, OFF_BN = OFF_TICKET + 16;
  __shared__ __attribute__((aligned(1024))) unsigned char smem_raw[OFF_BN + (xform ? 2 * MAX_BN_C * 4 : 0)];
  float* const smem = reinterpret_cast<float*>(smem_raw);
  float (*const epi)[BN] = reinterpret_cast<float (*)[BN]>(smem_raw + OFF_EPI);
  int& s_ticket = *reinterpret_cast<int*>(smem_raw + OFF_TICKET);
  float* const bnS = reinterpret_cast<float*>(smem_raw + OFF_BN);
  float* const bnT = bnS + MAX_BN_C;
  bool was_last = false;

  const int tid = threadIdx.x;
  const int lane = tid & 63, wave = __builtin_amdgcn_readfirstlane(tid >> 6);
  const int wm = wave / WGN, wn = wave % WGN;
  unsigned lbx = blockIdx.x, lby = blockIdx.y, lbz = blockIdx.z;
  if (a.xcd_remap) {
    const unsigned inner = gridDim.y * gridDim.z;
    const unsigned sw = xcd_swizzle(blockIdx.x + gridDim.x * (blockIdx.y + gridDim.y * blockIdx.z), gridDim.x * inner);
    lbx = sw / inner;
    const unsigned rem = sw - lbx * inner;
    lby = rem % gridDim.y;
    lbz = rem / gridDim.y;
  }
  const int n0 = lby * BN;
  const int phase = lbz / a.nsplit;
  const int split = lbz - phase * a.nsplit;

  const TapWalk tw = tap_walk(a, phase);
  const int ntx = tw.ntx, ky0 = tw.ky0, kx0 = tw.kx0, kstep_y = tw.kstep_y, kstep_x = tw.kstep_x;
  const int dsgn = tw.dsgn, cy = tw.cy, cx = tw.cx, phy = tw.phy, phx = tw.phx;
  const int nkc = a.Ck / BKG;
  const int total_all = tw.nty * ntx * nkc;
  const __amdgpu_buffer_rsrc_t srdX = __builtin_amdgcn_make_buffer_rsrc((void*)a.X, 0, (int)a.x_bytes, 0x00020000);
  const __amdgpu_buffer_rsrc_t srdW = __builtin_amdgcn_make_buffer_rsrc((void*)a.W, 0, (int)a.w_bytes, 0x00020000);
  const int per_split = (total_all + a.nsplit - 1) / a.nsplit;
  const int it_beg = split * per_split;
  const int it_end = it_beg + per_split < total_all ? it_beg + per_split : total_all;
  const int total = it_end > it_beg ? it_end - it_beg : 0;

  const int l31 = lane & 31, lhi = lane >> 5;
  const bool do_relu_bn = a.relu_bn.mode != 0 && !a.mix;
  const int hw = a.Hq * a.Wq;

  if (xform) {
    for (int c = tid; c < a.Ck; c += NT) {
      const BnC k = bn_coef(a.bn_in, c);
      bnS[c] = k.scale;
      bnT[c] = k.shift;
    }
  }
  for (int c = tid; c < BN; c += NT) {
    const int n = n0 + c;
    BnC k = BnC{0.f, 0.f, 0.f, 0.f};
    if (n < a.Cn && (do_relu_bn || a.mix)) k = bn_coef(a.relu_bn, n);
    if (a.mix) { k.scale *= a.mix_a; k.shift *= a.mix_a; }
    epi[0][c] = k.mean; epi[1][c] = k.rstd; epi[2][c] = k.scale; epi[3][c] = k.shift;
    epi[4][c] = (n < a.Cn && a.bias) ? a.bias[n] : 0.f;
  }
  __syncthreads();
  constexpr int E_LPR = WN / 8, E_RPP = 64 / E_LPR, E_NPASS = 32 / E_RPP;
  const int c8 = lane % E_LPR, rsub = lane / E_LPR;
  const int ecol = wn * WN + c8 * 8;
  const int ncol = n0 + ecol;
  const bool ok_lo = ncol < a.Cn, ok_hi = ncol + 4 < a.Cn;
  float s1[8], s2[8];
#pragma unroll
  for (int e = 0; e < 8; ++e) s1[e] = s2[e] = 0.f;
  float* const stg = smem + wave * 32 * STG_LD;
  const unsigned lds_base = (unsigned)(uintptr_t)((lds_void_t*)smem_raw);

  unsigned voffB[B_INSTR];
#pragma unroll
  for (int i = 0; i < B_INSTR; ++i) {
    const int pc = i * NW + wave;
    if (w_nk) {
      const int r = 8 * pc + (lane >> 3);
      const int cq = (lane & 7) ^ ((r >> 1) & 7);
      const int n = n0 + r;
      voffB[i] = n < a.Cn ? ((unsigned)n * (unsigned)a.Cout_w + (unsigned)cq * 4u) * 4u : OOB;
    } else {
      const int k = B_RPP * pc + lane / B_LPR;
      const int n = n0 + (lane % B_LPR) * 4;
      voffB[i] = n < a.Cn ? ((unsigned)k * (unsigned)a.Cout_w + (unsigned)n) * 4u : OOB;
    }
  }
  unsigned aoff[TI][4];
#pragma unroll
  for (int i = 0; i < TI; ++i) {
    const int r = wm * WM + i * 32 + l31;
#pragma unroll
    for (int q = 0; q < 4; ++q) aoff[i][q] = (unsigned)r * 128u + (unsigned)(((2 * q + lhi) ^ ((r >> 1) & 7)) * 16);
  }
  unsigned boff[TJ][w_nk ? 4 : 1];
#pragma unroll
  for (int j = 0; j < TJ; ++j) {
    if (w_nk) {
      const int r = wn * WN + j * 32 + l31;
#pragma unroll
      for (int q = 0; q < (w_nk ? 4 : 1); ++q)
        boff[j][q] = (unsigned)A_BYTES + (unsigned)r * 128u + (unsigned)(((2 * q + lhi) ^ ((r >> 1) & 7)) * 16);
    } else {
      boff[j][0] = (unsigned)A_BYTES + (unsigned)(4 * lhi) * (unsigned)B_ROWB + (unsigned)(wn * WN + j * 32 + l31) * 4u;
    }
  }

  const long nMt = (a.rows_per_phase + BM - 1) / BM;
  for (long mt = lbx; mt < nMt; mt += gridDim.x) {
    const long m0 = mt * BM;

    int ry0[A_INSTR], rx0[A_INSTR], rbase[A_INSTR];
    unsigned cqA[A_INSTR];
    bool rvalid[A_INSTR];
#pragma unroll
    for (int i = 0; i < A_INSTR; ++i) {
      const int r = 8 * (i * NW + wave) + (lane >> 3);
      cqA[i] = (unsigned)(((lane & 7) ^ ((r >> 1) & 7)) * 16);
      const long m = m0 + r;
      rvalid[i] = m < a.rows_per_phase;
      const unsigned mm = rvalid[i] ? (unsigned)m : 0u;
      const int n = (int)(mm / (unsigned)hw);
      const int rem = (int)(mm - (unsigned)n * (unsigned)hw);
      const int qy = rem / a.Wq, qx = rem - qy * a.Wq;
      if (a.form == 0) { ry0[i] = qy * a.sh - a.ph; rx0[i] = qx * a.sw - a.pw; }
      else             { ry0[i] = qy + cy;          rx0[i] = qx + cx; }
      rbase[i] = (n * a.Hx + ry0[i]) * a.Wx + rx0[i];
    }

    int ld_tap = it_beg / nkc;
    int ld_kc = (it_beg - ld_tap * nkc) * BKG;
    bool tap_dirty = true;
    unsigned offA[A_INSTR], offW = 0;

    float4 ra[xform ? R : 1][xform ? A_INSTR : 1];
    bool pend_ok[xform ? R : 1][xform ? A_INSTR : 1];
    float4 psc[xform ? R : 1], psh[xform ? R : 1];
    unsigned sB_set[xform ? R : 1];
    bool okA[A_INSTR];
    auto issue = [&](auto bufc) {
      constexpr int buf = decltype(bufc)::value;
      if (tap_dirty) {
        const int jy = ld_tap / ntx, jx = ld_tap - jy * ntx;
        const int wtap = (ky0 + kstep_y * jy) * a.kw + (kx0 + kstep_x * jx);
        const int tapoff = dsgn * (jy * a.Wx + jx);
#pragma unroll
        for (int i = 0; i < A_INSTR; ++i) {
          const int iy = ry0[i] + dsgn * jy, ix = rx0[i] + dsgn * jx;
          const bool ok = rvalid[i] & ((unsigned)iy < (unsigned)a.Hx) & ((unsigned)ix < (unsigned)a.Wx);
          offA[i] = ok ? (unsigned)(rbase[i] + tapoff) * (unsigned)a.Ck * 4u + cqA[i] : OOB;
          okA[i] = ok;
        }
        offW = (unsigned)wtap * (unsigned)a.Cin_w * (unsigned)a.Cout_w * 4u;
        tap_dirty = false;
      }
      const unsigned sA = (unsigned)ld_kc * 4u;
      const unsigned sB = offW + (w_nk ? (unsigned)ld_kc * 4u : (unsigned)ld_kc * (unsigned)a.Cout_w * 4u);
      if constexpr (xform) {
        constexpr int set = buf;
        const int kch = ld_kc + (int)(cqA[0] >> 2);
        {
          u32x4 cs, ct;
          lds_load_coef2(cs, ct, lds_base + (unsigned)OFF_BN + (unsigned)kch * 4u, lds_base + (unsigned)OFF_BN + (unsigned)(MAX_BN_C + kch) * 4u);
          psc[set] = __builtin_bit_cast(float4, cs);
          psh[set] = __builtin_bit_cast(float4, ct);
        }
#pragma unroll
        for (int i = 0; i < A_INSTR; ++i) { ra[set][i] = bld4s(srdX, offA[i], sA); pend_ok[set][i] = okA[i]; }
        sB_set[set] = sB;
      } else {
        unsigned char* const stage = smem_raw + buf * STAGE_BYTES;
#pragma unroll
        for (int i = 0; i < A_INSTR; ++i) lds_dma16(srdX, stage + (i * NW + wave) * 1024, offA[i], sA);
#pragma unroll
        for (int i = 0; i < B_INSTR; ++i) lds_dma16(srdW, stage + A_BYTES + (i * NW + wave) * 1024, voffB[i], sB);
      }
      ld_kc += BKG;
      if (ld_kc >= a.Ck) { ld_kc = 0; ++ld_tap; tap_dirty = true; }
    };
    auto commit = [&](auto bufc, auto setc) {
      constexpr int buf = decltype(bufc)::value, set = xform ? decltype(setc)::value : 0;
      unsigned char* const stage = smem_raw + buf * STAGE_BYTES;
#pragma unroll
      for (int i = 0; i < A_INSTR; ++i) {
        const float4 v = ra[set][xform ? i : 0];
        float4 t;
        t.x = fmaxf(fmaf(v.x, psc[set].x, psh[set].x), 0.f); t.y = fmaxf(fmaf(v.y, psc[set].y, psh[set].y), 0.f);
        t.z = fmaxf(fmaf(v.z, psc[set].z, psh[set].z), 0.f); t.w = fmaxf(fmaf(v.w, psc[set].w, psh[set].w), 0.f);
        if (!pend_ok[set][xform ? i : 0]) t = make_float4(0.f, 0.f, 0.f, 0.f);
        lds_store_b128(lds_base + (unsigned)(buf * STAGE_BYTES + (i * NW + wave) * 1024) + (unsigned)lane * 16u, __builtin_bit_cast(u32x4, t));
      }
#pragma unroll
      for (int i = 0; i < B_INSTR; ++i) lds_dma16(srdW, stage + A_BYTES + (i * NW + wave) * 1024, voffB[i], sB_set[set]);
    };

    f32x16 acc[TI][TJ];
#pragma unroll
    for (int i = 0; i < TI; ++i)
#pragma unroll
      for (int j = 0; j < TJ; ++j)
#pragma unroll
        for (int r = 0; r < 16; ++r) acc[i][j][r] = 0.f;

    using I0 = std::integral_constant<int, 0>; using I1 = std::integral_constant<int, 1>;
    using I2 = std::integral_constant<int, 2>; using I3 = std::integral_constant<int, 3>;
    if constexpr (xform) {
      if (total > 0) issue(I0{});
      if constexpr (R == 2) { if (total > 1) issue(I1{}); }
      if (total > 0) commit(I0{}, I0{});
      if (total > R) issue(I0{});
      if constexpr (NSTAGE == 4) {
        if (total > 1) commit(I1{}, I1{});
        if (total > 1 + R) issue(I1{});
        if (total > 2) commit(I2{}, I0{});
        if (total > 2 + R) issue(I0{});
      }
    } else {
      if (total > 0) issue(I0{});
      if (NSTAGE >= 3 && total > 1) issue(I1{});
      if (NSTAGE >= 4 && total > 2) issue(I2{});
    }

    auto chunk = [&](int it, auto curc) {
      constexpr int cur = decltype(curc)::value;
      if constexpr (xform) {
        if (R == 2 && it + NSTAGE - 2 + R < total) wait_vmcnt<LPS>();
        else wait_vmcnt<0>();
        asm volatile("s_waitcnt lgkmcnt(0)" ::: "memory");
      } else {
        const int younger = total - 1 - it < NSTAGE - 2 ? total - 1 - it : NSTAGE - 2;
        if (NSTAGE >= 4 && younger == 2) wait_vmcnt<2 * LPS>();
        else if (NSTAGE >= 3 && younger == 1) wait_vmcnt<LPS>();
        else wait_vmcnt<0>();
      }
      __builtin_amdgcn_sched_barrier(0);
      __builtin_amdgcn_s_barrier();
      __builtin_amdgcn_sched_barrier(0);
      if constexpr (xform) {
        constexpr int cbuf = (cur + NSTAGE - 1) % NSTAGE, cset = (cur + NSTAGE - 1) % R;
        if (it + NSTAGE - 1 < total) commit(std::integral_constant<int, cbuf>{}, std::integral_constant<int, cset>{});
// ... 402 lines not shown
```

### mopoe-mimic_amd/csrc/conv_gemm_glds_emu.inc

```
{
  static_assert(!xform, "EMU: plain operand forms");
  constexpr int NM = 6 * TI * TJ;
  constexpr int NP = 4 * (TI + TJ);
  f32x4v ea[2][TI], eb[2][w_nk ? TJ : 1];
  float ek[2][w_nk ? 1 : TJ][4];
  Split3 sa[2][TI], sb[2][TJ];

  auto top = [&](int it, auto curc) {
    constexpr int cur = decltype(curc)::value;
    const int younger = total - 1 - it < NSTAGE - 2 ? total - 1 - it : NSTAGE - 2;
    if (NSTAGE >= 4 && younger == 2) wait_vmcnt<2 * LPS>();
    else if (NSTAGE >= 3 && younger == 1) wait_vmcnt<LPS>();
    else wait_vmcnt<0>();
    __builtin_amdgcn_sched_barrier(0);
    __builtin_amdgcn_s_barrier();
    __builtin_amdgcn_sched_barrier(0);
    if (it + NSTAGE - 1 < total) issue(std::integral_constant<int, (cur + NSTAGE - 1) % NSTAGE>{});
  };
  auto reads = [&](auto curc, auto pc) {
    constexpr unsigned stage_off = (unsigned)(decltype(curc)::value * STAGE_BYTES);
    constexpr int p = decltype(pc)::value;
    static_for<2>([&](auto sc) {
      constexpr int s = decltype(sc)::value, q = 2 * p + s;
#pragma unroll
      for (int i = 0; i < TI; ++i) lds_frag_f4<0>(ea[s][i], lds_base + stage_off + aoff[i][q]);
      if constexpr (w_nk) {
#pragma unroll
        for (int j = 0; j < TJ; ++j) lds_frag_f4<0>(eb[s][w_nk ? j : 0], lds_base + stage_off + boff[j][w_nk ? q : 0]);
      } else {
#pragma unroll
        for (int j = 0; j < TJ; ++j) {
          lds_frag_f1<(8 * q + 0) * B_ROWB>(ek[s][w_nk ? 0 : j][0], lds_base + stage_off + boff[j][0]);
          lds_frag_f1<(8 * q + 1) * B_ROWB>(ek[s][w_nk ? 0 : j][1], lds_base + stage_off + boff[j][0]);
          lds_frag_f1<(8 * q + 2) * B_ROWB>(ek[s][w_nk ? 0 : j][2], lds_base + stage_off + boff[j][0]);
          lds_frag_f1<(8 * q + 3) * B_ROWB>(ek[s][w_nk ? 0 : j][3], lds_base + stage_off + boff[j][0]);
        }
      }
    });
  };
  auto fence_e = [&]() {
    MOPOE_DEVICE_ASM("s_waitcnt lgkmcnt(0)" ::: "memory");
#pragma unroll
    for (int s = 0; s < 2; ++s) {
#pragma unroll
      for (int i = 0; i < TI; ++i) pin_reg(ea[s][i]);
      if constexpr (w_nk) {
#pragma unroll
        for (int j = 0; j < TJ; ++j) pin_reg(eb[s][w_nk ? j : 0]);
      } else {
#pragma unroll
        for (int j = 0; j < TJ; ++j)
#pragma unroll
          for (int e = 0; e < 4; ++e) pin_reg(ek[s][w_nk ? 0 : j][e]);
      }
    }
    __builtin_amdgcn_sched_barrier(0);
  };
  auto piece = [&](auto uc, auto dc) {
    constexpr int u = decltype(uc)::value, d = decltype(dc)::value;
    constexpr int f = u / 4, w = u % 4, s = w / 2, e0 = 2 * (w % 2);
    unsigned h, m, l;
    if constexpr (f < TI) {
      split3_pair(ea[s][f][e0], ea[s][f][e0 + 1], h, m, l);
      sa[d][f].h[w] = h; sa[d][f].m[w] = m; sa[d][f].l[w] = l;
    } else {
      constexpr int j = f - TI;
      if constexpr (w_nk) split3_pair(eb[s][w_nk ? j : 0][e0], eb[s][w_nk ? j : 0][e0 + 1], h, m, l);
      else split3_pair(ek[s][w_nk ? 0 : j][e0], ek[s][w_nk ? 0 : j][e0 + 1], h, m, l);
      sb[d][j].h[w] = h; sb[d][j].m[w] = m; sb[d][j].l[w] = l;
    }
  };
  auto mfma_t = [&](auto tc, auto dc) {
    constexpr int t = decltype(tc)::value, d = decltype(dc)::value;
    constexpr int term = t / (TI * TJ), tile = t % (TI * TJ), i = tile % TI, j = tile / TI;
    mfma_split_term<term>(acc[i][j], sa[d][i], sb[d][j]);
  };
  using E0 = std::integral_constant<int, 0>; using E1 = std::integral_constant<int, 1>;
  auto all_pieces = [&](auto dc) { static_for<NP>([&](auto uc) { piece(uc, dc); }); };
  auto all_mfma = [&](auto dc) { static_for<NM>([&](auto tc) { mfma_t(tc, dc); }); };
  auto chunk2 = [&](int it, auto curc) {
    top(it, curc);
    reads(curc, E0{});
    fence_e();
    all_pieces(E0{});
    __builtin_amdgcn_sched_barrier(0);
    reads(curc, E1{});
    all_mfma(E0{});
    __builtin_amdgcn_sched_barrier(0);
    fence_e();
    all_pieces(E1{});
    __builtin_amdgcn_sched_barrier(0);
    all_mfma(E1{});
    __builtin_amdgcn_sched_barrier(0);
  };
  int it = 0;
  while (it < total) {
    chunk2(it, std::integral_constant<int, 0>{});
    if (++it >= total) break;
    chunk2(it, std::integral_constant<int, 1>{});
    if (++it >= total) break;
    if constexpr (NSTAGE >= 3) { chunk2(it, std::integral_constant<int, 2 % NSTAGE>{}); if (++it >= total) break; }
    if constexpr (NSTAGE >= 4) { chunk2(it, std::integral_constant<int, 3 % NSTAGE>{}); ++it; }
  }
}
```

### mopoe-mimic_amd/csrc/gemm_glds_common.inc

```
#pragma once

typedef __attribute__((address_space(3))) void lds_void_t;

template <int... Ns, typename F>
__device__ __forceinline__ void static_for_impl(std::integer_sequence<int, Ns...>, F&& f) { (f(std::integral_constant<int, Ns>{}), ...); }
template <int N, typename F>
__device__ __forceinline__ void static_for(F&& f) { static_for_impl(std::make_integer_sequence<int, N>{}, f); }

template <int N>
__device__ __forceinline__ void wait_vmcnt() {
  static_assert(N >= 0 && N <= 63, "vmcnt is a 6-bit counter");
  if constexpr (N == 0) asm volatile("s_waitcnt vmcnt(0)" ::: "memory");
  else if constexpr (N == 2) asm volatile("s_waitcnt vmcnt(2)" ::: "memory");
  else if constexpr (N == 3) asm volatile("s_waitcnt vmcnt(3)" ::: "memory");
  else if constexpr (N == 4) asm volatile("s_waitcnt vmcnt(4)" ::: "memory");
  else if constexpr (N == 5) asm volatile("s_waitcnt vmcnt(5)" ::: "memory");
  else if constexpr (N == 6) asm volatile("s_waitcnt vmcnt(6)" ::: "memory");
  else if constexpr (N == 7) asm volatile("s_waitcnt vmcnt(7)" ::: "memory");
  else if constexpr (N == 8) asm volatile("s_waitcnt vmcnt(8)" ::: "memory");
  else if constexpr (N == 10) asm volatile("s_waitcnt vmcnt(10)" ::: "memory");
  else if constexpr (N == 12) asm volatile("s_waitcnt vmcnt(12)" ::: "memory");
  else if constexpr (N == 14) asm volatile("s_waitcnt vmcnt(14)" ::: "memory");
  else if constexpr (N == 16) asm volatile("s_waitcnt vmcnt(16)" ::: "memory");
  else if constexpr (N == 24) asm volatile("s_waitcnt vmcnt(24)" ::: "memory");
  else static_assert(N == 0, "add the literal for this count");
}

#if defined(__HIP_DEVICE_COMPILE__)
#define MOPOE_DEVICE_ASM(...) asm volatile(__VA_ARGS__)
#define MOPOE_DEVICE_ASM_PURE(...) asm(__VA_ARGS__)
#else
#define MOPOE_DEVICE_ASM(...) do { } while (0)
#define MOPOE_DEVICE_ASM_PURE(...) do { } while (0)
#endif
__device__ __forceinline__ void lds_dma16(__amdgpu_buffer_rsrc_t srd, unsigned char* lds_dst, unsigned voff, unsigned soff) {
#if defined(__HIP_DEVICE_COMPILE__)
  __builtin_amdgcn_raw_ptr_buffer_load_lds(srd, (lds_void_t*)lds_dst, 16, voff, soff, 0, 0);
#endif
}

__device__ __forceinline__ void lds_store_b128(unsigned addr, u32x4 v) {
  MOPOE_DEVICE_ASM("ds_write_b128 %0, %1" :: "v"(addr), "v"(v) : "memory");
}
__device__ __forceinline__ void lds_load_coef2(u32x4& a, u32x4& b, unsigned addr_a, unsigned addr_b) {
  MOPOE_DEVICE_ASM("ds_read_b128 %0, %2\n\tds_read_b128 %1, %3\n\ts_waitcnt lgkmcnt(0)" : "=&v"(a), "=&v"(b) : "v"(addr_a), "v"(addr_b) : "memory");
}
__device__ __forceinline__ void lds_load_coef4(u32x4& a, u32x4& b, u32x4& c, u32x4& d, unsigned addr_a, unsigned addr_c) {
  MOPOE_DEVICE_ASM("ds_read_b128 %0, %4\n\tds_read_b128 %1, %4 offset:16\n\tds_read_b128 %2, %5\n\tds_read_b128 %3, %5 offset:16\n\ts_waitcnt lgkmcnt(0)"
                   : "=&v"(a), "=&v"(b), "=&v"(c), "=&v"(d) : "v"(addr_a), "v"(addr_c) : "memory");
}
```

### mopoe-mimic_amd/mimic_amd/layout.py

```python
from __future__ import annotations

import math
from typing import Tuple

import torch
import torch.nn as nn


def pack_weight(w_ref: torch.Tensor, kind: str) -> torch.Tensor:
    if kind == "linear":
        return w_ref.t().reshape(1, w_ref.shape[1], w_ref.shape[0]).contiguous()
    nk = w_ref.dim() - 2
    kdims = tuple(range(2, 2 + nk))
    if kind == "conv":
        p = w_ref.permute(*kdims, 1, 0)
    else:
        p = w_ref.permute(*kdims, 0, 1)
    return p.reshape(-1, p.shape[-2], p.shape[-1]).contiguous()


def unpack_weight(wp: torch.Tensor, kind: str, k: Tuple[int, ...]) -> torch.Tensor:
    taps, cin, cout = wp.shape
    if kind == "linear":
        return wp.reshape(cin, cout).t().contiguous()
# ... 7 lines not shown
class PackedConv(nn.Module):

    def __init__(self, cin: int, cout: int, k: Tuple[int, ...], kind: str, bias: bool):
        super().__init__()
        assert kind in ("conv", "convT", "linear")
        self.cin, self.cout, self.k, self.kind = cin, cout, tuple(k), kind
        taps = math.prod(k) if k else 1
        self.weight = nn.Parameter(torch.empty(taps, cin, cout))
        self.bias = nn.Parameter(torch.empty(cout)) if bias else None
        self.reset_parameters()

    def reset_parameters(self):
        taps = self.weight.shape[0]
        fan_in = (self.cout if self.kind == "convT" else self.cin) * taps
        bound = 1.0 / math.sqrt(fan_in)
        with torch.no_grad():
            self.weight.uniform_(-bound, bound)
            if self.bias is not None:
                self.bias.uniform_(-bound, bound)

    def ref_weight(self) -> torch.Tensor:
        return unpack_weight(self.weight.detach(), self.kind, self.k)

    def ref_grad(self):
        return None if self.weight.grad is None else unpack_weight(self.weight.grad, self.kind, self.k)

    def _save_to_state_dict(self, destination, prefix, keep_vars):
        destination[prefix + "weight"] = self.ref_weight()
        if self.bias is not None:
            destination[prefix + "bias"] = self.bias if keep_vars else self.bias.detach()

    def _load_from_state_dict(self, state_dict, prefix, local_metadata, strict, missing_keys, unexpected_keys,
                              error_msgs):
        key = prefix + "weight"
        if key in state_dict:
            w = state_dict[key]
            expect = tuple(unpack_weight(torch.empty(self.weight.shape, device="meta"), self.kind, self.k).shape)
            if tuple(w.shape) == expect:
                state_dict[key] = pack_weight(w, self.kind)
        super()._load_from_state_dict(state_dict, prefix, local_metadata, strict, missing_keys, unexpected_keys,
                                      error_msgs)


_param_epoch = [0]


def note_params_changed():
    _param_epoch[0] += 1


def param_epoch() -> int:
    return _param_epoch[0]


class Bf16Weights:

    def __init__(self, mods):
        self.mods = list(mods)
        self.flat = None
        self.views = {}
        self.versions = None
        self.synced_by_optimizer = False

    def _build(self):
        dev = self.mods[0].weight.device
        total = sum(-(-m.weight.numel() // 8) * 8 for m in self.mods)
        self.flat = torch.empty(total, dtype=torch.bfloat16, device=dev)
        off = 0
        for m in self.mods:
            n = m.weight.numel()
            self.views[id(m)] = self.flat[off:off + n].view(m.weight.shape)
            off += -(-n // 8) * 8
        self.versions = None

    def refresh(self, force: bool):
        if self.flat is None or self.flat.device != self.mods[0].weight.device:
            self._build()
        if self.synced_by_optimizer:
            force, vers = False, (None, [m.weight._version for m in self.mods])
        else:
            vers = (param_epoch(), [m.weight._version for m in self.mods])
        if force or vers != self.versions:
            with torch.no_grad():
                torch._foreach_copy_([self.views[id(m)] for m in self.mods], [m.weight.detach() for m in self.mods])
            self.versions = vers

    def bind_optimizer(self, on: bool):
        self.synced_by_optimizer = False
        self.versions = None
        if not on:
            return {}
        self.refresh(True)
        self.synced_by_optimizer = True
        self.versions = (None, [m.weight._version for m in self.mods])
        return {id(m.weight): self.views[id(m)].view(-1) for m in self.mods}

    def get(self, mod):
        return self.views[id(mod)]

    def has(self, mod):
        return id(mod) in self.views or any(m is mod for m in self.mods)


class BnParams(nn.Module):

    def __init__(self, c: int):
        super().__init__()
        self.weight = nn.Parameter(torch.ones(c))
        self.bias = nn.Parameter(torch.zeros(c))
        self.register_buffer("running_mean", torch.zeros(c))
        self.register_buffer("running_var", torch.ones(c))
        self.register_buffer("num_batches_tracked", torch.zeros((), dtype=torch.long))
        self.pending_batches = 0

    def _save_to_state_dict(self, destination, prefix, keep_vars):
        if self.pending_batches:
            self.num_batches_tracked += self.pending_batches
            self.pending_batches = 0
        super()._save_to_state_dict(destination, prefix, keep_vars)

    def _load_from_state_dict(self, state_dict, prefix, local_metadata, strict, missing_keys, unexpected_keys,
                              error_msgs):
        self.pending_batches = 0
        super()._load_from_state_dict(state_dict, prefix, local_metadata, strict, missing_keys, unexpected_keys,
                                      error_msgs)


class Indexed(nn.Module):

    def __init__(self, *mods):
        super().__init__()
        for i, m in enumerate(mods):
            self.add_module(str(i), m)

    def __getitem__(self, i):
        return self._modules[str(i)]

    def __len__(self):
        return len(self._modules)


class ResBlockParams(nn.Module):

    def __init__(self, cin: int, cout: int, k: Tuple[int, ...], transposed: bool, main_bias: bool, short_name: str):
        super().__init__()
        kind = "convT" if transposed else "conv"
        self.conv1 = PackedConv(cin, cin, (1,) * len(k), kind, main_bias)
        self.bn1 = BnParams(cin)
        self.bn2 = BnParams(cin)
        self.conv2 = PackedConv(cin, cout, k, kind, main_bias)
        self.add_module(short_name, Indexed(PackedConv(cin, cout, k, kind, True), BnParams(cout)))
        self.short_name = short_name

    @property
    def short(self):
        return self._modules[self.short_name]
```

### mopoe-mimic_amd/mimic_amd/nets.py

```python
from __future__ import annotations

from typing import Dict, List

import torch
import torch.nn as nn

import os

from . import ops
from .lanes import ModalityLanes
from .layout import Bf16Weights, BnParams, Indexed, PackedConv, ResBlockParams, param_epoch
from .ops import Geom
from .trunk import (BackwardArena, BlockSpec, MaskSource, StatsArena, apply_running_updates, stats_needed,
                    trunk_backward, trunk_forward)


def _lin_geom(cin, cout):
    return Geom(1, 1, 1, 1, 1, cin, cout, 1, 1, 1, 1, 0, 0, False)


class _NetFn(torch.autograd.Function):

    @staticmethod
    def forward(ctx, net, n_in, *tensors):
        inputs = tensors[:n_in]
        if ops.STAMPS is not None:
            ops.stamp(f"{type(net).__name__}#{id(net) % 997} fwd begin")
        outs, saved = net._run_forward(*inputs)
        if ops.STAMPS is not None:
            ops.stamp(f"{type(net).__name__}#{id(net) % 997} fwd end")
        ctx.net, ctx.saved, ctx.n_in = net, saved, n_in
        ctx.in_needs_grad = [isinstance(t, torch.Tensor) and t.requires_grad for t in inputs]
        return outs if isinstance(outs, tuple) else (outs,)

    @staticmethod
    def backward(ctx, *gouts):
        net = ctx.net
        from .plugins import is_zero_placeholder
        gouts = [None if g is None else (g if is_zero_placeholder(g) else g.contiguous()) for g in gouts]
        if ops.STAMPS is not None:
            ops.stamp(f"{type(net).__name__}#{id(net) % 997} bwd begin")
        gin, grads, arena = net._run_backward(ctx.saved, ctx.in_needs_grad, *gouts)
        if ops.STAMPS is not None:
            ops.stamp(f"{type(net).__name__}#{id(net) % 997} bwd end")
        ctx.saved = None
        plist = [grads.get(name) for name, _ in net._named_param_list()]
        reducer = getattr(net, "_grad_reducer", None)
        if reducer is not None:
            reducer.network_done(arena, [g for g in plist if g is not None])
        return (None, None, *gin, *plist)


class _GroupFn(torch.autograd.Function):

    @staticmethod
    def forward(ctx, group, *tensors):
        lanes = ModalityLanes(tensors[0].device)
        outs_all, saved_all, needs_all, off = [], [], [], 0
        order = _group_order(group, 0)
        spans = []
        for net, name, n_in, n_par in group:
            spans.append((off, off + n_in))
            off += n_in + n_par
        res = [None] * len(group)
        for i in order:
            net, name, n_in, n_par = group[i]
            inputs = tensors[spans[i][0]:spans[i][1]]
            lanes.share(*[t for t in inputs if torch.is_tensor(t)])
            with lanes.fork(name):
                if ops.STAMPS is not None:
                    ops.stamp(f"{type(net).__name__}:{name} fwd begin")
                outs, saved = net._run_forward(*inputs)
                if ops.STAMPS is not None:
                    ops.stamp(f"{type(net).__name__}:{name} fwd end")
            outs = outs if isinstance(outs, tuple) else (outs,)
            res[i] = (outs, saved, [isinstance(t, torch.Tensor) and t.requires_grad for t in inputs])
        lanes.join(*[t for r in res for t in r[0] if torch.is_tensor(t)])
        ctx.group, ctx.saved, ctx.needs = group, [r[1] for r in res], [r[2] for r in res]
        ctx.n_out = [len(r[0]) for r in res]
        return tuple(t for r in res for t in r[0])

    @staticmethod
    def backward(ctx, *gouts):
        from .plugins import is_zero_placeholder
        group = ctx.group
        gouts = [None if g is None else (g if is_zero_placeholder(g) else g.contiguous()) for g in gouts]
        dev = next(g.device for g in gouts if g is not None)
        lanes = ModalityLanes(dev)
        lanes.share(*[g for g in gouts if g is not None])
        per, off = [], 0
        for n in ctx.n_out:
            per.append(gouts[off:off + n])
            off += n
        order = _group_order(group, 1)
# ... 11 lines not shown
                if reducer is not None:
                    reducer.network_done(arena, [g for g in plist if g is not None])
                elif EARLY_STEP[0] is not None:
                    EARLY_STEP[0]([p for _, p in net._named_param_list()], plist, inline=not lanes.forks(name))
            res[i] = (*gin, *plist)
        ctx.saved = None
        lanes.join(*[t for r in res for t in r if torch.is_tensor(t)])
        return (None, *[t for r in res for t in r])


GROUP_TEXT = os.environ.get("MOPOE_GROUP_TEXT", "first,first").split(",")


def _group_order(group, phase):
    first = GROUP_TEXT[phase] == "first"
    return sorted(range(len(group)), key=lambda i: (group[i][1] != "text") == first)


EARLY_STEP = [None]


GROUP_NODES = os.environ.get("MOPOE_GROUP_NODES", "1") != "0"


def run_group(items):
    if len(items) < 2 or not GROUP_NODES:
        lanes, outs = None, []
        for name, net, args in items:
            first = next(a for a in args if torch.is_tensor(a))
            if lanes is None:
                lanes = ModalityLanes(first.device)
            lanes.share(*[a for a in args if torch.is_tensor(a)])
            with lanes.fork(name):
                outs.append(net(*args))
        if lanes is not None:
            lanes.join(*[t for o in outs for t in o if torch.is_tensor(t)])
        return outs
    group, tensors = [], []
    for name, net, args in items:
        inputs = net._group_inputs(*args)
        params = [p for _, p in net._named_param_list()]
        group.append((net, name, len(inputs), len(params)))
        tensors += [*inputs, *params]
    flat = _GroupFn.apply(group, *tensors)
    outs, off = [], 0
    for (name, net, args), n in zip(items, [len(net._out_names) for _, net, _ in items]):
        outs.append(net._finish(tuple(flat[off:off + n])))
        off += n
    return outs


def compute_dtype(flags):
    name = str(getattr(flags, "compute_dtype", "fp32")).lower()
    if name in ("bf16", "bfloat16"):
        return torch.bfloat16
    if name in ("fp32", "f32", "float32"):
        return torch.float32
    raise ValueError(f"compute_dtype must be 'fp32' or 'bf16', not {name!r}")


class _HipNet(nn.Module):

    mask_source: MaskSource = MaskSource()

    def _misc_numel(self) -> int:
        n = getattr(self, "_misc_numel_cache", None)
        if n is None:
            trunk = set()
            for spec in self.blocks:
                trunk.update(id(p) for p in spec.params.parameters())
            n = sum(p.numel() + 4 for p in self.parameters() if id(p) not in trunk)
            object.__setattr__(self, "_misc_numel_cache", n)
        return n
    dropout_enabled = True
    act_dtype = torch.float32
    _shadow = None

    def _init_dtype(self, flags, fp32_mods=()):
        self.act_dtype = compute_dtype(flags)
        if self.act_dtype == torch.bfloat16:
            keep = {id(m) for m in fp32_mods}
            mods = [m for m in self.modules() if isinstance(m, PackedConv) and id(m) not in keep]
            object.__setattr__(self, "_shadow", Bf16Weights(mods))

    def _begin_forward(self):
        if self._shadow is not None:
            self._shadow.refresh(self.training)

    def _w(self, mod):
        if self._shadow is not None and self._shadow.has(mod):
            return self._shadow.get(mod)
        return mod.weight

    def _bf16(self):
        return self.act_dtype == torch.bfloat16

    def _named_param_list(self):
        if getattr(self, "_plist", None) is None:
            self._plist = [(n, p) for n, p in self.named_parameters()]
        return self._plist

    def _call(self, *inputs):
        params = [p for _, p in self._named_param_list()]
        return _NetFn.apply(self, len(inputs), *inputs, *params)

    def _dropout_on(self):
        return self.training and self.dropout_enabled

    def _arena(self, blocks, device):
        return StatsArena(stats_needed(blocks), device, self.training)


class _FeatureExtractorImg(nn.Module):
    def __init__(self, flags):
        super().__init__()
        d, s = flags.DIM_img, flags.img_size
        self.conv1 = PackedConv(flags.image_channels, d, (3, 3), "conv", False)
        plan = [(d, 2 * d, 2, 1), (2 * d, 3 * d, 2, 1), (3 * d, 4 * d, 2, 1)]
        if s == 64:
            plan += [(4 * d, 5 * d, 2, 0)]
        elif s == 128:
            plan += [(4 * d, 5 * d, 2, 1), (5 * d, 5 * d, 2, 0)]
        elif s == 256:
            plan += [(4 * d, 5 * d, 4, 1), (5 * d, 5 * d, 2, 0)]
        else:
            raise AttributeError("img_size must be one of 64, 128, 256")
        self.plan = plan
        for i, (ci, co, _st, _pd) in enumerate(plan):
            self.add_module(f"resblock_{i + 1}", Indexed(ResBlockParams(ci, co, (4, 4), False, False, "downsample")))


class _Compressor(nn.Module):

    def __init__(self, cin, style_dim, cout):
        super().__init__()
        if style_dim:
            raise NotImplementedError("factorized_representation / style latents are out of scope (SURVEY §2.1-4)")
        self.style_mu = None
        self.style_logvar = None
        self.content_mu = PackedConv(cin, cout, (), "linear", True)
        self.content_logvar = PackedConv(cin, cout, (), "linear", True)


def _compress_fwd(comp: _Compressor, feat, batch, w=lambda m: m.weight):
    g = _lin_geom(comp.content_mu.cin, comp.content_mu.cout).with_batch(batch)
    mu = ops.conv_fwd(feat, w(comp.content_mu), g, bias=comp.content_mu.bias, out_dtype=torch.float32)
    lv = ops.conv_fwd(feat, w(comp.content_logvar), g, bias=comp.content_logvar.bias, out_dtype=torch.float32)
    return mu.view(batch, -1), lv.view(batch, -1), g


def _compress_bwd(comp: _Compressor, feat, g, gmu, glv, grads, prefix, w=lambda m: m.weight, arena=None):
    batch = feat.shape[0]
    dfeat = None
    take = (lambda shape: arena.take_misc(shape)) if arena is not None else (lambda shape: None)
    for name, mod, gg in (("content_mu", comp.content_mu, gmu), ("content_logvar", comp.content_logvar, glv)):
        if gg is None:
            continue
        gg4 = gg.reshape(batch, 1, 1, -1)
        grads[f"{prefix}.{name}.bias"] = ops.colsum(gg4, out=take((gg4.shape[-1],)))
        if feat.dtype != gg4.dtype:
            gg4 = gg4.to(feat.dtype)
        grads[f"{prefix}.{name}.weight"] = ops.conv_wgrad(feat, gg4, g, out=take((g.taps, g.Cin, g.Cout)))
        d = ops.conv_dgrad(gg4, w(mod), g, out_dtype=torch.float32)
        dfeat = d if dfeat is None else dfeat.add_(d)
    return dfeat if dfeat is None or dfeat.dtype == feat.dtype else dfeat.to(feat.dtype)

# ... 490 lines not shown
```

### mopoe-mimic_amd/mimic_amd/ops.py

```python
from __future__ import annotations

import ctypes as C
import os
from dataclasses import dataclass
from functools import lru_cache
from typing import Optional, Sequence

import torch

_HERE = os.path.dirname(os.path.abspath(__file__))
LIB_PATH = os.environ.get("MOPOE_HIP_LIB") or os.path.join(os.path.dirname(_HERE), "csrc", "libmopoe_hip.so")
ABI_VERSION = 20

RES_A, RES_B = 2.0, 0.3
BN_EPS = 1e-5
SUBSET_MASKS = (1, 2, 4, 3, 5, 6, 7)


class MopoeHipError(RuntimeError):
    pass


class _Geom(C.Structure):
    _fields_ = [(n, C.c_int32) for n in
                ("N", "Hs", "Ws", "Hb", "Wb", "Cin", "Cout", "kh", "kw", "sh", "sw", "ph", "pw", "transposed")]


class _BnRef(C.Structure):
    _fields_ = [("sums", C.c_void_p), ("gamma", C.c_void_p), ("beta", C.c_void_p), ("rmean", C.c_void_p),
                ("rvar", C.c_void_p), ("inv_count", C.c_double), ("eps", C.c_float), ("C", C.c_int32),
                ("mode", C.c_int32)]


class _MaskRef(C.Structure):
    _fields_ = [("mask", C.c_void_p), ("kind", C.c_int32), ("rows_per_sample", C.c_int32)]


class _MixRef(C.Structure):
    _fields_ = [("s", C.c_void_p), ("bn", _BnRef), ("a", C.c_float), ("b", C.c_float)]


class _RunDesc(C.Structure):
    _fields_ = [("sums", C.c_void_p), ("rmean", C.c_void_p), ("rvar", C.c_void_p), ("C", C.c_int32),
                ("count", C.c_int32)]


class _AdamSeg(C.Structure):
    _fields_ = [("p", C.c_void_p), ("g", C.c_void_p), ("m", C.c_void_p), ("v", C.c_void_p), ("p16", C.c_void_p),
                ("n", C.c_int64)]


@dataclass(frozen=True)
class Geom:
    N: int
    Hs: int
    Ws: int
    Hb: int
    Wb: int
    Cin: int
    Cout: int
    kh: int
    kw: int
    sh: int
    sw: int
    ph: int
    pw: int
    transposed: bool

    def __post_init__(self):
        object.__setattr__(self, "_hash", hash((self.N, self.Hs, self.Ws, self.Hb, self.Wb, self.Cin, self.Cout, self.kh,
                                                self.kw, self.sh, self.sw, self.ph, self.pw, self.transposed)))

    def __hash__(self):
        return self._hash

    @property
    def in_shape(self):
        return (self.N, self.Hs, self.Ws, self.Cin) if self.transposed else (self.N, self.Hb, self.Wb, self.Cin)

    @property
    def out_shape(self):
        return (self.N, self.Hb, self.Wb, self.Cout) if self.transposed else (self.N, self.Hs, self.Ws, self.Cout)

    @property
    def taps(self):
        return self.kh * self.kw

    def with_batch(self, n):
        return _with_batch(self, n)

    def c(self):
        return _geom_struct(self)


@lru_cache(maxsize=None)
def _with_batch(g: "Geom", n: int) -> "Geom":
    return Geom(n, *[getattr(g, f) for f in
                     ("Hs", "Ws", "Hb", "Wb", "Cin", "Cout", "kh", "kw", "sh", "sw", "ph", "pw", "transposed")])


@lru_cache(maxsize=None)
def _geom_struct(g: "Geom") -> "_Geom":
    return _Geom(g.N, g.Hs, g.Ws, g.Hb, g.Wb, g.Cin, g.Cout, g.kh, g.kw, g.sh, g.sw, g.ph, g.pw, int(g.transposed))


@dataclass
class Bn:
    gamma: torch.Tensor
    beta: torch.Tensor
    mode: int
    sums: Optional[torch.Tensor] = None
    count: int = 0
    rmean: Optional[torch.Tensor] = None
    rvar: Optional[torch.Tensor] = None
    eps: float = BN_EPS

    def c(self):
        return _BnRef(_p(self.sums), _p(self.gamma), _p(self.beta), _p(self.rmean), _p(self.rvar),
                      (1.0 / self.count) if self.count else 0.0, self.eps, self.gamma.numel(), self.mode)


@dataclass
class Mask:
    mask: torch.Tensor
    kind: int
    rows_per_sample: int = 1

    def c(self):
        return _MaskRef(_p(self.mask), self.kind, self.rows_per_sample)


_NO_BN = _BnRef(None, None, None, None, None, 0.0, 0.0, 0, 0)
_NO_MASK = _MaskRef(None, 0, 1)


def _p(t: Optional[torch.Tensor]):
    return None if t is None else C.c_void_p(t.data_ptr())


_lib = None


def lib():
    global _lib
    if _lib is None:
        if not os.path.exists(LIB_PATH):
            raise MopoeHipError(f"{LIB_PATH} not built: run `python __graft_entry__.py build` "
                                "(mimic_amd has no CPU fallback)")
        _lib = C.CDLL(LIB_PATH)
        _lib.mopoe_last_error.restype = C.c_char_p
        _lib.mopoe_abi_version.restype = C.c_int
        if _lib.mopoe_abi_version() != ABI_VERSION:
            raise MopoeHipError("libmopoe_hip.so ABI version mismatch")
    return _lib


def _check(rc: int):
    if rc != 0:
        raise MopoeHipError(f"libmopoe_hip error {rc}: {lib().mopoe_last_error().decode()}")


_raw_stream = getattr(torch._C, "_cuda_getCurrentRawStream", None)


def _stream_ptr(device=None) -> int:
    if _raw_stream is not None:
        idx = torch.cuda.current_device() if device is None or device.index is None else device.index
        return _raw_stream(idx)
    return torch.cuda.current_stream(device).cuda_stream


def _stream():
    return C.c_void_p(_stream_ptr())


def _dev(*ts):
    for t in ts:
        if t is not None:
            if not t.is_cuda:
                raise MopoeHipError("mimic_amd ops need GPU tensors (no CPU fallback)")
            if not t.is_contiguous():
                raise MopoeHipError("mimic_amd ops need contiguous tensors")


def _bn(bn: Optional[Bn]):
    return C.byref(bn.c()) if bn is not None else C.byref(_NO_BN)


def _mask(m: Optional[Mask]):
    return C.byref(m.c()) if m is not None else C.byref(_NO_MASK)


_conv_ws = {}


def _workspace(device):
    key = (device.index, _stream_ptr(device))
    if key not in _conv_ws:
        lib().mopoe_conv_workspace_bytes.restype = C.c_size_t
        nbytes = int(lib().mopoe_conv_workspace_bytes())
        _conv_ws[key] = (torch.zeros(nbytes, dtype=torch.uint8, device=device), nbytes)
    return _conv_ws[key]


def new_stats(n_channels: int, device) -> torch.Tensor:
    return torch.zeros(2, n_channels, dtype=torch.float64, device=device)


class _Plan(C.Structure):
    _fields_ = [("tile", C.c_int32), ("split", C.c_int32)]


AUTOTUNE = os.environ.get("MOPOE_AUTOTUNE", "1") not in ("0", "table")
TABLE_ONLY = os.environ.get("MOPOE_AUTOTUNE", "1") == "table"
_TUNE_REPS = int(os.environ.get("MOPOE_TUNE_REPS", "3"))
TUNE_AFTER_CALLS = int(os.environ.get("MOPOE_TUNE_AFTER_CALLS", "0"))
TUNE_ALPHA = float(os.environ.get("MOPOE_TUNE_ALPHA", "0.7"))
DIRECT_TILES = os.environ.get("MOPOE_DIRECT_TILES", "0") != "0"
_conv_calls = 0
_plans = {}
_GATHER_TILES = ((128, 128), (256, 64), (64, 64), (256, 128), (128, 64), (64, 64), (128, 64), (128, 128),
                 (128, 128), (256, 64), (64, 64), (128, 64),
                 (128, 128), (128, 64), (64, 64), (256, 128),
                 (128, 128), (128, 64), (64, 64), (256, 128))
F32_GLDS = os.environ.get("MOPOE_F32_GLDS", "1") != "0"
F32_SPLIT_BF16 = os.environ.get("MOPOE_F32_SPLIT_BF16", "1") != "0"
_SPLITS = (2, 3, 4, 6, 8, 12, 16, 24, 32, 48, 64, 96, 128)


_forced_plan = None

PLAN_TABLE_PATH = os.environ.get("MOPOE_PLAN_TABLE", os.path.join(os.path.dirname(os.path.abspath(__file__)), "plans_gfx950.json"))
USE_PLAN_TABLE = os.environ.get("MOPOE_AUTOTUNE", "1") != "force" and os.environ.get("MOPOE_PLAN_TABLE", "") != "0"
_plan_table = None


def plan_key_str(key) -> str:
    g = key[1]
    geo = ",".join(str(int(getattr(g, f))) for f in ("N", "Hs", "Ws", "Hb", "Wb", "Cin", "Cout", "kh", "kw", "sh", "sw", "ph", "pw", "transposed"))
    return f"{key[0]}|{geo}|" + ",".join(str(int(f)) if isinstance(f, bool) else str(f) for f in key[2:])


def _table_plan(key):
    global _plan_table
    if _plan_table is None:
        _plan_table = {}
        if USE_PLAN_TABLE and os.path.exists(PLAN_TABLE_PATH):
            import json
            with open(PLAN_TABLE_PATH) as f:
                _plan_table = json.load(f).get("plans", {})
    v = _plan_table.get(plan_key_str(key), False)
    if v is False and key[0] in ("fwd", "fwd16") and len(key) >= 4 and isinstance(key[3], bool):
        v = _plan_table.get(plan_key_str(key[:3] + (not key[3],) + key[4:]), False)
    if v is False:
        return False, None
    if v is not None and not F32_SPLIT_BF16:
        if key[0] in ("fwd", "dgrad") and v[0] >= 16:
            v = [v[0] - 4, v[1]]
        elif key[0] == "wgrad" and v[0] in (7, 8):
            v = [v[0] - 2, v[1]]
        elif key[0] == "wgrad" and v[0] in (9, 10):
            v = [2, v[1]]
    return True, (None if v is None else _Plan(int(v[0]), int(v[1])))


_plan_sources = {"table": 0, "tuned": 0, "static": 0}


def plan_source_summary():
    return dict(_plan_sources, table_file=os.path.basename(PLAN_TABLE_PATH) if USE_PLAN_TABLE and os.path.exists(PLAN_TABLE_PATH) else None)


def clear_plans():
    _plans.clear()


class force_plan:

    def __init__(self, tile: int, split: int):
        self.plan = _Plan(tile, split)

    def __enter__(self):
        global _forced_plan
        self.prev, _forced_plan = _forced_plan, self.plan
        return self

    def __exit__(self, *exc):
        global _forced_plan
        _forced_plan = self.prev


_plan_log = {}

# ... 194 lines not shown
    cands = {}
    for tile, (bm, bn) in enumerate(_GATHER_TILES_BF16):
        blocks = -(-rows // bm) * -(-cn // bn) * nphase
        if bm == 256 and rows < 256:
            continue
        if tile >= 5 and not (BF16_GLDS and ck % 64 == 0 and tile in _GLDS_TILES and (plain_operand or tile in (5, 7, 9, 11))):
            continue
        if tile >= 5 and taps * (ck // 64) < 2:
            continue
        cap = _GLDS_TILES[tile] if tile >= 5 else (512 if tile == 3 else 768)
        cands[(tile, 1)] = min(1.0, blocks / cap)
        for sp in _SPLITS:
            if sp * 2 <= iters and blocks * sp <= 2048 and sp * per <= ws_bytes:
                cands[(tile, sp)] = min(1.0, blocks * sp / cap)
    return cands


def conv_mix_supported(x, g: Geom) -> bool:
    return _is16(x) or (g.Cin % 4 == 0 and g.Cout % 4 == 0)


def conv_fwd(x, wp, g: Geom, bn_in: Optional[Bn] = None, bias=None, mask: Optional[Mask] = None,
             out_stats=None, out_dtype=None, mix=None):
    _dev(x, wp, bias, out_stats)
    assert tuple(x.shape) == g.in_shape and tuple(wp.shape) == (g.taps, g.Cin, g.Cout)
    out_dtype = out_dtype or x.dtype
    gc = g.c()
    stream = _stream()
    mixr = None
    if mix is not None:
        ms, mbn = mix[0], mix[1]
        _dev(ms)
        assert tuple(ms.shape) == g.out_shape and ms.dtype == out_dtype and ms.is_contiguous() and conv_mix_supported(x, g)
        mixc = _MixRef(ms.data_ptr(), mbn.c(), float(mix[2]) if len(mix) > 2 else RES_A, float(mix[3]) if len(mix) > 3 else RES_B)
        mixr = C.byref(mixc)
    if _is16(x) or out_dtype == BF16:
        plain = bn_in is None and mask is None
        if not g.transposed and g.Cin == 1:
            assert plain and bias is None and x.dtype == torch.float32 and wp.dtype == torch.float32
            y = torch.empty(g.out_shape, dtype=BF16, device=x.device)
            _check(lib().mopoe_edge_expand_bf16(_p(x), _p(wp), _p(y), C.byref(gc), g.Cout, _p(out_stats), stream))
            return y
        if g.transposed and g.Cout == 1:
            assert plain and out_stats is None and _is16(x) and wp.dtype == torch.float32
            y = torch.empty(g.out_shape, dtype=torch.float32, device=x.device)
            _check(lib().mopoe_edge_reduce_bf16(_p(x), _p(wp), _p(bias), _p(y), C.byref(gc), g.Cin, stream))
            return y
        if not (_is16(x) and _is16(wp)):
            raise MopoeHipError("bf16 conv needs a bf16 activation and the bf16 copy of the packed weight")
        y = torch.empty(g.out_shape, dtype=out_dtype, device=x.device)
        ws, nbytes = _workspace(x.device)
        fn = lib().mopoe_conv_fwd_bf16
        bnr, mr, f32 = _bn(bn_in), _mask(mask), C.c_int32(int(out_dtype == torch.float32))

        def launch16(plan, stats=None):
            if mixr is not None:
                _check(lib().mopoe_conv_fwd_mix_bf16(_p(x), _p(wp), _p(bias), _p(y), C.byref(gc), bnr, mr, mixr, _p(stats),
                                                     plan, _p(ws), C.c_size_t(nbytes), stream))
                return
            _check(fn(_p(x), _p(wp), _p(bias), _p(y), f32, C.byref(gc), bnr, mr, _p(stats), plan, _p(ws),
                      C.c_size_t(nbytes), stream))

        key = ("fwd16", g, bn_in is not None, mask is not None, out_stats is not None, out_dtype) + (("mix",) if mix is not None else ())
        plan = _tuned_plan(key, lambda: _gather_candidates_bf16("fwd", g, nbytes, plain_operand=bn_in is None),
                           lambda ref: launch16(ref, _scratch_like(out_stats)))
        launch16(plan, out_stats)
        return y
    y = torch.empty(g.out_shape, dtype=torch.float32, device=x.device)
    ws, nbytes = _workspace(x.device)
    fn = lib().mopoe_conv_fwd
    bnr, mr = _bn(bn_in), _mask(mask)

    def launch(plan, stats=None):
        if mixr is not None:
            _check(lib().mopoe_conv_fwd_mix(_p(x), _p(wp), _p(bias), _p(y), C.byref(gc), bnr, mr, mixr, _p(stats), plan,
                                            _p(ws), C.c_size_t(nbytes), stream))
            return
        _check(fn(_p(x), _p(wp), _p(bias), _p(y), C.byref(gc), bnr, mr, _p(stats), plan, _p(ws), C.c_size_t(nbytes),
                  stream))

    key = ("fwd", g, bn_in is not None, mask is not None, out_stats is not None) + (("mix",) if mix is not None else ())
    plan = _tuned_plan(key, lambda: _gather_candidates("fwd", g, nbytes, plain_operand=bn_in is None),
                       lambda ref: launch(ref, _scratch_like(out_stats)))
    launch(plan, out_stats)
    return y


def conv_dgrad(dy, wp, g: Geom, relu_bn: Optional[Bn] = None, xin=None, bwd_sums=None, out_dtype=None):
    _dev(dy, wp, xin, bwd_sums)
    assert tuple(dy.shape) == g.out_shape
    out_dtype = out_dtype or dy.dtype
    gc = g.c()
    stream = _stream()
    if _is16(dy) or out_dtype == BF16:
        if g.transposed and g.Cout == 1:
            assert relu_bn is None and dy.dtype == torch.float32 and wp.dtype == torch.float32
            dx = torch.empty(g.in_shape, dtype=BF16, device=dy.device)
            _check(lib().mopoe_edge_expand_bf16(_p(dy), _p(wp), _p(dx), C.byref(gc), g.Cin, None, stream))
            return dx
        if not (_is16(dy) and _is16(wp)) or (xin is not None and not _is16(xin)):
            raise MopoeHipError("bf16 conv_dgrad needs bf16 dy / xin and the bf16 copy of the packed weight")
        dx = torch.empty(g.in_shape, dtype=out_dtype, device=dy.device)
        ws, nbytes = _workspace(dy.device)
        fn = lib().mopoe_conv_dgrad_bf16
        bnr, f32 = _bn(relu_bn), C.c_int32(int(out_dtype == torch.float32))

        def launch16(plan, sums=None):
            _check(fn(_p(dy), _p(wp), _p(dx), f32, C.byref(gc), bnr, _p(xin), _p(sums), plan, _p(ws), C.c_size_t(nbytes),
                      stream))

        key = ("dgrad16", g, relu_bn is not None, bwd_sums is not None, out_dtype)
        plan = _tuned_plan(key, lambda: _gather_candidates_bf16("dgrad", g, nbytes, plain_operand=True),
                           lambda ref: launch16(ref, _scratch_like(bwd_sums)))
        launch16(plan, bwd_sums)
        return dx
    dx = torch.empty(g.in_shape, dtype=torch.float32, device=dy.device)
    ws, nbytes = _workspace(dy.device)
    fn = lib().mopoe_conv_dgrad
    bnr = _bn(relu_bn)

    def launch(plan, sums=None):
        _check(fn(_p(dy), _p(wp), _p(dx), C.byref(gc), bnr, _p(xin), _p(sums), plan, _p(ws), C.c_size_t(nbytes), stream))

    key = ("dgrad", g, relu_bn is not None, bwd_sums is not None)
    plan = _tuned_plan(key, lambda: _gather_candidates("dgrad", g, nbytes, plain_operand=True),
                       lambda ref: launch(ref, _scratch_like(bwd_sums)))
    launch(plan, bwd_sums)
    return dx


def conv_wgrad(x, dy, g: Geom, bn_in: Optional[Bn] = None, out=None):
    _dev(x, dy, out)
    assert tuple(x.shape) == g.in_shape and tuple(dy.shape) == g.out_shape
    dwp = out if out is not None else torch.empty((g.taps, g.Cin, g.Cout), dtype=torch.float32, device=x.device)
    assert tuple(dwp.shape) == (g.taps, g.Cin, g.Cout) and dwp.dtype == torch.float32
    gc = g.c()
    stream = _stream()
    bnr = _bn(bn_in)
    if _is16(x) or _is16(dy):
        if min(g.Cin, g.Cout) == 1:
            assert bn_in is None
            vec, scal = (dy, x) if g.Cin == 1 else (x, dy)
            assert _is16(vec) and scal.dtype == torch.float32
            _check(lib().mopoe_edge_wgrad_bf16(_p(vec), _p(scal), _p(dwp), C.byref(gc), max(g.Cin, g.Cout),
                                               C.c_int32(int(out is not None)), stream))
            return dwp
        if not (_is16(x) and _is16(dy)):
            raise MopoeHipError("bf16 conv_wgrad needs both operands in bf16")
        fn = lib().mopoe_conv_wgrad_bf16
        key = ("wgrad16", g, bn_in is not None)
    else:
        fn = lib().mopoe_conv_wgrad
        key = ("wgrad", g, bn_in is not None)

    def launch(plan, dst, is_zero):
        _check(fn(_p(x), _p(dy), _p(dst), C.byref(gc), bnr, C.c_int32(is_zero), plan, stream))

    plan = _tuned_plan(key, lambda: _wgrad_candidates(g, bf16=key[0] == "wgrad16", plain_operand=bn_in is None),
                       lambda ref: launch(ref, _scratch_like(dwp), 1))
    launch(plan, dwp, int(out is not None))
    return dwp


def _rows(t):
    return t.numel() // t.shape[-1]


def block_out_fwd(s, m, bn_s: Bn, a=RES_A, b=RES_B, out_stats=None):
    _dev(s, m, out_stats)
    out = torch.empty_like(s)
    fn = lib().mopoe_block_out_fwd_bf16 if _is16(s) else lib().mopoe_block_out_fwd
    _check(fn(_p(s), _p(m), _p(out), C.c_int64(_rows(s)), s.shape[-1], _bn(bn_s),
                                     C.c_float(a), C.c_float(b), _p(out_stats), _stream()))
    return out


def bn_relu_apply(x, bn: Bn):
    _dev(x)
    out = torch.empty_like(x)
    fn = lib().mopoe_bn_relu_apply_bf16 if _is16(x) else lib().mopoe_bn_relu_apply
    _check(fn(_p(x), _p(out), C.c_int64(_rows(x)), x.shape[-1], _bn(bn), _stream()))
    return out


BLOCK_FRONT = os.environ.get("MOPOE_BLOCK_FRONT", "1") != "0"
BLOCK_FRONT_F32 = os.environ.get("MOPOE_BLOCK_FRONT_F32", "1") != "0"
BLOCK_FRONT_F32_FWD = os.environ.get("MOPOE_BLOCK_FRONT_F32_FWD", "0") != "0"


def block_front_supported(x, g1: "Geom", mask1: Optional[Mask], forward: bool = False) -> bool:
    if forward and not _is16(x) and not BLOCK_FRONT_F32_FWD:
        return False
    return (BLOCK_FRONT and x.dtype in (BF16, torch.float32) and (_is16(x) or BLOCK_FRONT_F32) and g1.Cin == 64 and g1.Cout == 64
            and g1.taps == 1 and _rows(x) % 32 == 0
            and (mask1 is None or (mask1.kind == 1 and mask1.rows_per_sample % 32 == 0)))


def block_front_stats(x, w1, bias, bn1: Bn, mask1: Optional[Mask], out_stats):
    _dev(x, w1, bias, out_stats)
    fn = lib().mopoe_block_front_stats_bf16 if _is16(x) else lib().mopoe_block_front_stats
    _check(fn(_p(x), _p(w1), _p(bias), C.c_int64(_rows(x)), x.shape[-1], _bn(bn1), _mask(mask1),
                                              _p(out_stats), _stream()))
    return out_stats


def block_front_apply(x, w1, bias, bn1: Bn, bn2: Bn, mask1: Optional[Mask]):
    _dev(x, w1, bias)
    a2 = torch.empty_like(x)
    fn = lib().mopoe_block_front_apply_bf16 if _is16(x) else lib().mopoe_block_front_apply
    _check(fn(_p(x), _p(w1), _p(bias), _p(a2), C.c_int64(_rows(x)), x.shape[-1], _bn(bn1), _bn(bn2),
# ... 5 lines not shown
                    dbeta2=None):
    _dev(x, dh2, w1, bias, sums2, sums1, dw1, dbias, dgamma2, dbeta2)
    dh1 = torch.empty_like(x)
    fn = lib().mopoe_block_front_bwd_bf16 if _is16(x) else lib().mopoe_block_front_bwd
    _check(fn(_p(x), _p(dh2), _p(w1), _p(bias), _p(dh1), C.c_int64(_rows(x)), x.shape[-1], _bn(bn1),
                                            _bn(bn2), _mask(mask1), _p(sums2), _p(sums1), _p(dw1), _p(dbias), _p(dgamma2), _p(dbeta2),
                                            _stream()))
    return dh1


def bn_bwd_reduce(g, s, bn_s: Bn, sums=None):
    _dev(g, s, sums)
    if sums is None:
        sums = new_stats(s.shape[-1], s.device)
    fn = lib().mopoe_bn_bwd_reduce_bf16 if _is16(s) else lib().mopoe_bn_bwd_reduce
    _check(fn(_p(g), _p(s), C.c_int64(_rows(s)), s.shape[-1], _bn(bn_s), _p(sums), _stream()))
    return sums


def block_out_bwd(g, s, bn_s: Bn, sums, mask: Optional[Mask], a=RES_A, b=RES_B, want_colsum_dm=False,
                  want_colsum_ds=True, small=None):
    _dev(g, s, sums)
    c = s.shape[-1]
    dm, ds = torch.empty_like(g), torch.empty_like(g)
    if small is None:
        small = torch.zeros(4, c, dtype=torch.float32, device=g.device)
    cdm = small[2] if want_colsum_dm else None
    cds = small[3] if want_colsum_ds else None
    fn = lib().mopoe_block_out_bwd_bf16 if _is16(s) else lib().mopoe_block_out_bwd
    _check(fn(_p(g), _p(s), _p(dm), _p(ds), C.c_int64(_rows(s)), c, _bn(bn_s), _p(sums), _mask(mask), C.c_float(a),
              C.c_float(b), _p(small[0]), _p(small[1]), _p(cdm), _p(cds), _stream()))
    return dm, ds, small[0], small[1], cdm, cds


def bn_bwd_apply(dy, x, bn: Bn, sums, mask: Optional[Mask] = None, add=None, want_colsum=False, small=None,
                 next_s=None, next_bn: Optional[Bn] = None, next_sums=None):
    _dev(dy, x, sums, add, next_s, next_sums)
    c = x.shape[-1]
    dx = torch.empty_like(x)
    if small is None:
        small = torch.zeros(3, c, dtype=torch.float32, device=x.device)
    cs = small[2] if want_colsum else None
    nb = _bn(next_bn) if next_s is not None else None
    fn = lib().mopoe_bn_bwd_apply_bf16 if _is16(x) else lib().mopoe_bn_bwd_apply
    _check(fn(_p(dy), _p(x), _p(add), _p(dx), C.c_int64(_rows(x)), c, _bn(bn), _p(sums), _mask(mask), _p(small[0]),
              _p(small[1]), _p(cs), _p(next_s), nb, _p(next_sums), _stream()))
    return dx, small[0], small[1], cs


def bn_running_update(entries: Sequence, momentum=0.1):
    entries = list(entries)
    if not entries:
        return
    arr = (_RunDesc * len(entries))()
    for i, (sums, rm, rv, count) in enumerate(entries):
        _dev(sums, rm, rv)
        arr[i] = _RunDesc(sums.data_ptr(), rm.data_ptr(), rv.data_ptr(), rm.numel(), count)
    _check(lib().mopoe_bn_running_update(arr, len(entries), C.c_float(momentum), _stream()))


STAMPS = None


def stamp(name):
    st = STAMPS
    if st is None:
        return
    if "buf" not in st:
        st["buf"] = torch.zeros(256, dtype=torch.int64, device="cuda")
        st["names"] = []
    i = len(st["names"])
    if i >= st["buf"].numel():
        return
    st["names"].append(name)
    _check(lib().mopoe_prof_stamp(C.c_void_p(st["buf"].data_ptr() + 8 * i), _stream()))


def adam_step(params, grads, ms, vs, step, lr, beta1, beta2, eps, coef, lowp=None, prep=True):
    n = len(params)
    arr = (_AdamSeg * n)()
    for i in range(n):
        p_, g_ = params[i], grads[i]
        if g_ is None:
            arr[i] = _AdamSeg(p_.data_ptr(), None, ms[i].data_ptr(), vs[i].data_ptr(), None, p_.numel())
            continue
        if g_.dtype != torch.float32 or p_.dtype != torch.float32 or g_.numel() != p_.numel():
            raise MopoeHipError("adam_step: parameters and gradients must be fp32 tensors of equal size")
        _dev(p_, g_, ms[i], vs[i])
        lp = lowp[i] if lowp is not None else None
        arr[i] = _AdamSeg(p_.data_ptr(), g_.data_ptr(), ms[i].data_ptr(), vs[i].data_ptr(),
                          None if lp is None else lp.data_ptr(), p_.numel())
    lr_dev = lr if isinstance(lr, torch.Tensor) else None
    _check(lib().mopoe_adam_step(arr, n, _p(step) if prep else None, _p(lr_dev), C.c_double(0.0 if lr_dev is not None else float(lr)),
                                 C.c_double(beta1), C.c_double(beta2), C.c_double(eps), _p(coef), _stream()))


def colsum(x, out=None):
    _dev(x, out)
    zero = out is not None
    if out is None:
        out = torch.empty(x.shape[-1], dtype=torch.float32, device=x.device)
    assert out.dtype == torch.float32 and out.numel() == x.shape[-1]
    fn = lib().mopoe_colsum_bf16 if _is16(x) else lib().mopoe_colsum
    _check(fn(_p(x), _p(out), C.c_int64(_rows(x)), x.shape[-1], C.c_int32(int(zero)), _stream()))
    return out


def _ptr3(ts):
    arr = (C.c_void_p * 3)()
    for i, t in enumerate(ts):
        arr[i] = None if t is None else t.data_ptr()
    return arr


_kl_ws = {}


def _ws(device, n=8):
    key = (device.index, n, _stream_ptr(device) if device.type == "cuda" else 0)
    if key not in _kl_ws:
        _kl_ws[key] = torch.zeros(n, dtype=torch.float64, device=device)
    return _kl_ws[key]


def latent_fwd(mu_in, lv_in, eps, row_start, w, norm):
    present = [t for t in mu_in if t is not None]
    _dev(*present, *[t for t in lv_in if t is not None], eps)
    b, d = present[0].shape
    k = len(row_start) - 1
    dev = present[0].device
    mus = torch.empty(k, b, d, dtype=torch.float32, device=dev)
    lvs = torch.empty_like(mus)
    jm, jl, z = (torch.empty(b, d, dtype=torch.float32, device=dev) for _ in range(3))
    klds = torch.empty(k, dtype=torch.float32, device=dev)
    jd = torch.empty(1, dtype=torch.float32, device=dev)
    rs = (C.c_int32 * (k + 1))(*row_start)
    wa = (C.c_float * k)(*w)
    _check(lib().mopoe_latent_fwd(_ptr3(mu_in), _ptr3(lv_in), _p(eps), b, d, rs, wa, C.c_float(norm), _p(mus),
                                  _p(lvs), _p(jm), _p(jl), _p(z), _p(klds), _p(jd), _p(_ws(dev)),
                                  _stream()))
    return mus, lvs, jm, jl, z, klds, jd


def latent_bwd(mu_in, lv_in, eps, row_start, w, norm, g_mus, g_lvs, g_jm, g_jl, g_z, g_klds, g_jd):
    present = [t for t in mu_in if t is not None]
    _dev(*present, eps, *[t for t in (g_mus, g_lvs, g_jm, g_jl, g_z, g_klds, g_jd) if t is not None])
    b, d = present[0].shape
    dmu = [None if t is None else torch.empty_like(t) for t in mu_in]
    dlv = [None if t is None else torch.empty_like(t) for t in lv_in]
    k = len(row_start) - 1
    rs = (C.c_int32 * (k + 1))(*row_start)
    wa = (C.c_float * k)(*w)
    _check(lib().mopoe_latent_bwd(_ptr3(mu_in), _ptr3(lv_in), _p(eps), b, d, rs, wa, C.c_float(norm), _p(g_mus),
                                  _p(g_lvs), _p(g_jm), _p(g_jl), _p(g_z), _p(g_klds), _p(g_jd), _ptr3(dmu),
                                  _ptr3(dlv), _stream()))
    return dmu, dlv


LATENT_METHODS = {"moe": 0, "jsd": 1}


def _mixture_args(method, mu_in, member_row_start, comp_row_start, w):
    if method not in LATENT_METHODS:
        raise MopoeHipError(f"latent_mixture: method must be one of {sorted(LATENT_METHODS)}, not {method!r}")
    n = sum(t is not None for t in mu_in)
    c = n + (method == "jsd")
    if len(comp_row_start) != c + 1 or len(w) != c:
        raise MopoeHipError(f"latent_mixture: {method} with {n} modalities takes {c} components")
    flat = [v for part in member_row_start for v in (list(part) + [0] * 4)[:4]]
    if len(flat) != 12:
        raise MopoeHipError("latent_mixture: member_row_start holds the partitions over 1, 2 and 3 members")
    return (LATENT_METHODS[method], c, (C.c_int32 * 12)(*flat), (C.c_int32 * (c + 1))(*comp_row_start),
            (C.c_float * c)(*w))


def latent_mixture_fwd(method, mu_in, lv_in, eps, member_row_start, comp_row_start, w, norm):
    present = [t for t in mu_in if t is not None]
# ... 252 lines not shown
```

Before: 6515.

## Presplit fp32 conv weights into bf16 hi/mid/lo planes for emulated GEMM

New measurement: 6576, median of 6. Within noise of the previous version (+0.9%).

```diff
diff --git a/include/mopoe_hip.h b/include/mopoe_hip.h
--- a/include/mopoe_hip.h
+++ b/include/mopoe_hip.h
@@ -8,7 +8,7 @@
 extern "C" {
 #endif
 
-#define MOPOE_ABI_VERSION 20
+#define MOPOE_ABI_VERSION 21
 
 #define MOPOE_OK 0
 #define MOPOE_ERR_ARG (-1)
@@ -52,6 +52,7 @@
 typedef struct {
   int32_t tile;
   int32_t split;
+  const uint16_t* wplanes;
 } mopoe_conv_plan;
 
 int mopoe_conv_fwd(const float* x, const float* wp, const float* bias, float* y,
@@ -231,11 +232,19 @@
   float* m;
   float* v;
   uint16_t* p16;
+  uint16_t* planes;
   int64_t n;
 } mopoe_adam_seg;
 int mopoe_adam_step(const mopoe_adam_seg* segs, int32_t nseg, float* step, const float* lr_dev, double lr, double beta1,
                     double beta2, double eps, float* coef, void* stream);
 
+typedef struct {
+  const float* w;
+  uint16_t* planes;
+  int64_t n;
+} mopoe_split_seg;
+int mopoe_split_planes(const mopoe_split_seg* segs, int32_t nseg, void* stream);
+
 #define MOPOE_PROF_KINDS 144
 int mopoe_prof_enable(int32_t on);
 int mopoe_prof_stamp(uint64_t* slot, void* stream);
diff --git a/mopoe-mimic_amd/csrc/adam.hip b/mopoe-mimic_amd/csrc/adam.hip
--- a/mopoe-mimic_amd/csrc/adam.hip
+++ b/mopoe-mimic_amd/csrc/adam.hip
@@ -1,6 +1,10 @@
-#include "common.hpp"
+#include <utility>
+
+#include "gemm_common.hpp"
 
 namespace mopoe {
+
+#include "split3.inc"
 
 constexpr int ADAM_SEGS_PER_LAUNCH = 64;
 constexpr int ADAM_CHUNK = 4096;
@@ -32,6 +36,20 @@
   v = (float)(h.beta2 * (double)v + (1.0 - h.beta2) * (double)g * (double)g);
   const float denom = (float)((double)(sqrtf(v) / h.bc2_sqrt) + h.eps);
   p -= h.step_size * m / denom;
+}
+
+__device__ __forceinline__ void store_planes4(uint16_t* planes, long n, long e, const float4& p) {
+  unsigned h0, m0, l0, h1, m1, l1;
+  split3_pair(p.x, p.y, h0, m0, l0);
+  split3_pair(p.z, p.w, h1, m1, l1);
+  *reinterpret_cast<uint2*>(planes + e) = make_uint2(h0, h1);
+  *reinterpret_cast<uint2*>(planes + n + e) = make_uint2(m0, m1);
+  *reinterpret_cast<uint2*>(planes + 2 * n + e) = make_uint2(l0, l1);
+}
+__device__ __forceinline__ void store_planes1(uint16_t* planes, long n, long e, float p) {
+  unsigned h, m, l;
+  split3_pair(p, 0.f, h, m, l);
+  planes[e] = (uint16_t)h; planes[n + e] = (uint16_t)m; planes[2 * n + e] = (uint16_t)l;
 }
 
 __global__ __launch_bounds__(ADAM_THREADS) void adam_kernel(const AdamPack pack, int nseg, const float* __restrict__ coef,
@@ -49,7 +67,8 @@
   h.step_size = coef[0]; h.bc2_sqrt = coef[1];
 
   const bool vec = ((((uintptr_t)s.p | (uintptr_t)s.g | (uintptr_t)s.m | (uintptr_t)s.v) & 15) == 0) &&
-                   (s.p16 == nullptr || (((uintptr_t)s.p16) & 7) == 0);
+                   (s.p16 == nullptr || (((uintptr_t)s.p16) & 7) == 0) &&
+                   (s.planes == nullptr || ((((uintptr_t)s.planes) & 7) == 0 && (s.n & 3) == 0));
   if (vec) {
     float4 p[4], g[4], m[4], v[4];
     bool ok[4];
@@ -81,6 +100,7 @@
         o.y = pack_bf16(p[i].z, p[i].w);
         *reinterpret_cast<uint2*>(s.p16 + e) = o;
       }
+      if (s.planes) store_planes4(s.planes, s.n, e, p[i]);
     }
     const long tail = s.n & ~3L;
     if (tid == 0 && tail >= base && tail < base + ADAM_CHUNK) {
@@ -89,6 +109,7 @@
         adam_one(pp, s.g[e], mm, vv, h);
         s.p[e] = pp; s.m[e] = mm; s.v[e] = vv;
         if (s.p16) s.p16[e] = f32_to_bf16(pp);
+        if (s.planes) store_planes1(s.planes, s.n, e, pp);
       }
     }
   } else {
@@ -99,6 +120,35 @@
       adam_one(pp, s.g[e], mm, vv, h);
       s.p[e] = pp; s.m[e] = mm; s.v[e] = vv;
       if (s.p16) s.p16[e] = f32_to_bf16(pp);
+      if (s.planes) store_planes1(s.planes, s.n, e, pp);
+    }
+  }
+}
+
+struct SplitPack {
+  mopoe_split_seg seg[ADAM_SEGS_PER_LAUNCH];
+  int chunk_start[ADAM_SEGS_PER_LAUNCH];
+};
+__global__ __launch_bounds__(ADAM_THREADS) void split_planes_kernel(const SplitPack pack, int nseg) {
+  const int tid = threadIdx.x, lane = tid & 63;
+  const int b = (int)blockIdx.x;
+  const unsigned long long le = __ballot(pack.chunk_start[lane] <= b);
+  const int si = __builtin_amdgcn_readfirstlane(__popcll(le) - 1);
+  if (si < 0 || si >= nseg) return;
+  const mopoe_split_seg s = pack.seg[si];
+  const long base = (long)(b - pack.chunk_start[si]) * ADAM_CHUNK;
+  const bool vec = ((((uintptr_t)s.w) & 15) == 0) && ((((uintptr_t)s.planes) & 7) == 0) && (s.n & 3) == 0;
+  if (vec) {
+#pragma unroll
+    for (int i = 0; i < 4; ++i) {
+      const long e = base + (long)(i * ADAM_THREADS + tid) * 4;
+      if (e < s.n) store_planes4(s.planes, s.n, e, *reinterpret_cast<const float4*>(s.w + e));
+    }
+  } else {
+    for (int i = tid; i < ADAM_CHUNK; i += ADAM_THREADS) {
+      const long e = base + i;
+      if (e >= s.n) break;
+      store_planes1(s.planes, s.n, e, s.w[e]);
     }
   }
 }
@@ -139,3 +189,31 @@
   }
   return MOPOE_OK;
 }
+
+extern "C" int mopoe_split_planes(const mopoe_split_seg* segs, int32_t nseg, void* stream) {
+  if ((!segs && nseg != 0) || nseg < 0) { set_error("split_planes: bad arguments"); return MOPOE_ERR_ARG; }
+  hipStream_t st = (hipStream_t)stream;
+  int32_t i = 0;
+  while (i < nseg) {
+    SplitPack pack;
+    int n = 0;
+    long blocks = 0;
+    for (; i < nseg && n < ADAM_SEGS_PER_LAUNCH; ++i) {
+      const mopoe_split_seg& s = segs[i];
+      if (s.n == 0) continue;
+      if (!s.w || !s.planes || s.n < 0) { set_error("split_planes: record %d is incomplete", (int)i); return MOPOE_ERR_ARG; }
+      const long nb = (s.n + ADAM_CHUNK - 1) / ADAM_CHUNK;
+      if (nb > 0x7fffffffL) { set_error("split_planes: record %d has more than 2^43 elements", (int)i); return MOPOE_ERR_ARG; }
+      if (blocks + nb > 0x7fffffffL) break;
+      pack.seg[n] = s;
+      pack.chunk_start[n] = (int)blocks;
+      blocks += nb;
+      ++n;
+    }
+    for (int k = n; k < ADAM_SEGS_PER_LAUNCH; ++k) { pack.seg[k] = mopoe_split_seg{}; pack.chunk_start[k] = 0x7fffffff; }
+    if (n == 0) continue;
+    hipLaunchKernelGGL(split_planes_kernel, dim3((unsigned)blocks), dim3(ADAM_THREADS), 0, st, pack, n);
+    if (int rc = check_launch("split_planes")) return rc;
+  }
+  return MOPOE_OK;
+}
diff --git a/mopoe-mimic_amd/csrc/conv_gemm.hip b/mopoe-mimic_amd/csrc/conv_gemm.hip
--- a/mopoe-mimic_amd/csrc/conv_gemm.hip
+++ b/mopoe-mimic_amd/csrc/conv_gemm.hip
@@ -54,6 +54,8 @@
   int mix;
   float mix_a, mix_b;
   int xcd_remap;
+  const unsigned short* wplanes;
+  unsigned wpl_plane_bytes;
 };
 
 __device__ __forceinline__ float epi_round(const GemmArgs&, float x) { return x; }
@@ -1000,6 +1002,7 @@
                    (!xin || aligned16(xin)) && (!mask || mask->kind == 0 || aligned16(mask->mask));
   a.x_bytes = (unsigned)std::min<size_t>(xb, 0x7fffffffu);
   a.w_bytes = (unsigned)std::min<size_t>(wb, 0x7fffffffu);
+  a.wplanes = nullptr; a.wpl_plane_bytes = 0;
   mopoe_bn_ref none = {};
   mopoe_mask_ref nomask = {nullptr, 0, 1};
   a.bn_in = bn_in ? *bn_in : none;
@@ -1039,6 +1042,14 @@
       if (a.bn_in.mode != 0) { set_error("conv plan: tile %d (split-bf16 products) has no BN-on-load form", cfg); return MOPOE_ERR_ARG; }
       emu = true;
       cfg -= 4;
+      if (plan->wplanes && cfg != 12) {
+        if (3 * (wb / 2) >= (1ull << 31) || (((uintptr_t)plan->wplanes) & 15) != 0 || (wb / 2) % 16 != 0) {
+          set_error("conv plan: weight planes must be 16-byte aligned planes of < 2 GiB in all");
+          return MOPOE_ERR_ARG;
+        }
+        a.wplanes = plan->wplanes;
+        a.wpl_plane_bytes = (unsigned)(wb / 2);
+      }
     }
     if (cfg >= 12 && (!vec || Ck % 32 != 0 || (a.bn_in.mode != 0 && cfg == 13))) {
       set_error("conv plan: tile %d (LDS-DMA family) needs the vector path, K channels %% 32 == 0 (Ck = %d) and, with BN on load, tile 12, 14 or 15", cfg, Ck);
@@ -1111,13 +1122,24 @@
     if (spec == 1) hipLaunchKernelGGL((gather_gemm_f32_glds_kernel<BM_, BN_, WM_, WN_, 1, ST_, 1>), grid, dim3(64 * WM_ * WN_), 0, stream, a); \
     else hipLaunchKernelGGL((gather_gemm_f32_glds_kernel<BM_, BN_, WM_, WN_, 3, ST_, 1>), grid, dim3(64 * WM_ * WN_), 0, stream, a);          \
   } while (0)
-    if (emu) {
+#define MOPOE_LAUNCH_GLDS_EMU_WPL(BM_, BN_, WM_, WN_, ST_)                                                                               \
+  do {                                                                                                                                \
+    if (spec == 1) hipLaunchKernelGGL((gather_gemm_f32_glds_kernel<BM_, BN_, WM_, WN_, 1, ST_, 2>), grid, dim3(64 * WM_ * WN_), 0, stream, a); \
+    else hipLaunchKernelGGL((gather_gemm_f32_glds_kernel<BM_, BN_, WM_, WN_, 3, ST_, 2>), grid, dim3(64 * WM_ * WN_), 0, stream, a);          \
+  } while (0)
+    if (emu && a.wplanes) {
+      if (cfg == 13) MOPOE_LAUNCH_GLDS_EMU_WPL(128, 64, 2, 2, 2);
+      else if (cfg == 14) MOPOE_LAUNCH_GLDS_EMU_WPL(64, 64, 2, 2, 3);
+      else MOPOE_LAUNCH_GLDS_EMU_WPL(256, 128, 4, 2, 2);
+    }
+    else if (emu) {
       if (cfg == 12) MOPOE_LAUNCH_GLDS_EMU(128, 128, 2, 2, 2);
       else if (cfg == 13) MOPOE_LAUNCH_GLDS_EMU(128, 64, 2, 2, 3);
       else if (cfg == 14) MOPOE_LAUNCH_GLDS_EMU(64, 64, 2, 2, 4);
       else MOPOE_LAUNCH_GLDS_EMU(256, 128, 4, 2, 3);
     }
 #undef MOPOE_LAUNCH_GLDS_EMU
+#undef MOPOE_LAUNCH_GLDS_EMU_WPL
     else if (cfg >= 12) {
       if (spec == 2) {
         if (cfg == 12) hipLaunchKernelGGL((gather_gemm_f32_glds_kernel<128, 128, 2, 2, 2, 2>), grid, dim3(256), 0, stream, a);
diff --git a/mopoe-mimic_amd/csrc/conv_gemm_bf16_glds.inc b/mopoe-mimic_amd/csrc/conv_gemm_bf16_glds.inc
--- a/mopoe-mimic_amd/csrc/conv_gemm_bf16_glds.inc
+++ b/mopoe-mimic_amd/csrc/conv_gemm_bf16_glds.inc
@@ -15,11 +15,6 @@
 __device__ __forceinline__ void lds_frag_b128(bf16x8& r, unsigned addr) {
   static_assert(OFF >= 0 && OFF < 65536, "ds offset field");
   MOPOE_DEVICE_ASM("ds_read_b128 %0, %1 offset:%2" : "=v"(r) : "v"(addr), "n"(OFF) : "memory");
-}
-template <int OFF>
-__device__ __forceinline__ void lds_frag_tr64(s16x4& r, unsigned addr) {
-  static_assert(OFF >= 0 && OFF < 65536, "ds offset field");
-  MOPOE_DEVICE_ASM("ds_read_b64_tr_b16 %0, %1 offset:%2" : "=v"(r) : "v"(addr), "n"(OFF) : "memory");
 }
 template <int TI, int TJ>
 __device__ __forceinline__ void fence_frags(bf16x8 (&fa)[TI], bf16x8 (&fb)[TJ]) {
@@ -148,8 +143,7 @@
       voffB[i] = n < a.Cn ? ((unsigned)n * (unsigned)a.Cout_w + (unsigned)cq * 8u) * 2u : OOB;
     } else {
       const int k = B_RPP * pc + lane / B_LPR;
-      const int g = BN == 128 ? (k & 3) : ((k >> 1) & 1);
-      const int cq = (lane % B_LPR) ^ (g << 2);
+      const int cq = (lane % B_LPR) ^ kstrided_swz<BN>(k);
       const int n = n0 + cq * 8;
       voffB[i] = n < a.Cn ? ((unsigned)k * (unsigned)a.Cout_w + (unsigned)n) * 2u : OOB;
     }
@@ -173,8 +167,7 @@
       const int i16 = lane & 15, g16 = (lane >> 4) & 1;
       const int k = lhi * 8 + (i16 >> 2);
       const int colb = (wn * WN + j * 32 + g16 * 16 + (i16 & 3) * 4) * 2;
-      const int g = BN == 128 ? (k & 3) : ((k >> 1) & 1);
-      boff[j][0] = (unsigned)A_BYTES + (unsigned)k * (unsigned)B_ROWB + (unsigned)((((colb >> 4) ^ (g << 2)) << 4) | (colb & 15));
+      boff[j][0] = (unsigned)A_BYTES + (unsigned)k * (unsigned)B_ROWB + (unsigned)((((colb >> 4) ^ kstrided_swz<BN>(k)) << 4) | (colb & 15));
     }
   }
 
diff --git a/mopoe-mimic_amd/csrc/conv_gemm_glds.inc b/mopoe-mimic_amd/csrc/conv_gemm_glds.inc
--- a/mopoe-mimic_amd/csrc/conv_gemm_glds.inc
+++ b/mopoe-mimic_amd/csrc/conv_gemm_glds.inc
@@ -11,28 +11,7 @@
   MOPOE_DEVICE_ASM("ds_read_b32 %0, %1 offset:%2" : "=v"(r) : "v"(addr), "n"(OFF) : "memory");
 }
 
-typedef __bf16 e_bf16x2 __attribute__((ext_vector_type(2)));
-typedef __bf16 e_bf16x8 __attribute__((ext_vector_type(8)));
-typedef float e_f32x2 __attribute__((ext_vector_type(2)));
-struct Split3 { u32x4 h, m, l; };
-
-__device__ __forceinline__ void split3_pair(float a0, float a1, unsigned& h, unsigned& m, unsigned& l) {
-#if defined(MOPOE_DBG_EMU_NOSPLIT)
-  h = __float_as_uint(a0); m = __float_as_uint(a1); l = h;
-  return;
-#endif
-  const e_f32x2 a = {a0, a1};
-  h = __builtin_bit_cast(unsigned, __builtin_convertvector(a, e_bf16x2));
-  float r0 = 0.f, r1 = 0.f, q0 = 0.f, q1 = 0.f;
-  MOPOE_DEVICE_ASM_PURE("v_sub_f32 %0, %1, %2" : "=v"(r0) : "v"(a0), "v"(h << 16));
-  MOPOE_DEVICE_ASM_PURE("v_sub_f32 %0, %1, %2" : "=v"(r1) : "v"(a1), "v"(h & 0xffff0000u));
-  const e_f32x2 r = {r0, r1};
-  m = __builtin_bit_cast(unsigned, __builtin_convertvector(r, e_bf16x2));
-  MOPOE_DEVICE_ASM_PURE("v_sub_f32 %0, %1, %2" : "=v"(q0) : "v"(r0), "v"(m << 16));
-  MOPOE_DEVICE_ASM_PURE("v_sub_f32 %0, %1, %2" : "=v"(q1) : "v"(r1), "v"(m & 0xffff0000u));
-  const e_f32x2 r2 = {q0, q1};
-  l = __builtin_bit_cast(unsigned, __builtin_convertvector(r2, e_bf16x2));
-}
+#include "split3.inc"
 __device__ __forceinline__ void split3_first(float a0, float a1, unsigned& h, float& r0, float& r1) {
   const e_f32x2 a = {a0, a1};
   h = __builtin_bit_cast(unsigned, __builtin_convertvector(a, e_bf16x2));
@@ -103,8 +82,12 @@
   constexpr bool w_nk = SPEC == 3;
   constexpr int BKG = 32;
   constexpr int A_BYTES = BM * 128;
-  constexpr int B_ROWB = w_nk ? 128 : BN * 4;
-  constexpr int B_BYTES = BN * 128;
+  constexpr bool WPL = EMU == 2;
+  static_assert(!WPL || !xform, "weight planes: plain operand forms");
+  constexpr int W_ESZ = WPL ? 2 : 4;
+  constexpr int B_ROWB = w_nk ? 32 * W_ESZ : BN * W_ESZ;
+  constexpr int PLANE_BYTES = BN * 32 * W_ESZ;
+  constexpr int B_BYTES = WPL ? 3 * PLANE_BYTES : PLANE_BYTES;
   constexpr int STAGE_BYTES = A_BYTES + B_BYTES;
   constexpr int A_INSTR = A_BYTES / (NT * 16), B_INSTR = B_BYTES / (NT * 16);
   static_assert(A_BYTES % (NT * 16) == 0 && B_BYTES % (NT * 16) == 0 && A_INSTR >= 1 && B_INSTR >= 1, "whole 1-KB pieces per wave");
@@ -145,7 +128,8 @@
   const int nkc = a.Ck / BKG;
   const int total_all = tw.nty * ntx * nkc;
   const __amdgpu_buffer_rsrc_t srdX = __builtin_amdgcn_make_buffer_rsrc((void*)a.X, 0, (int)a.x_bytes, 0x00020000);
-  const __amdgpu_buffer_rsrc_t srdW = __builtin_amdgcn_make_buffer_rsrc((void*)a.W, 0, (int)a.w_bytes, 0x00020000);
+  const __amdgpu_buffer_rsrc_t srdW = WPL ? __builtin_amdgcn_make_buffer_rsrc((void*)a.wplanes, 0, (int)(3u * a.wpl_plane_bytes), 0x00020000)
+                                          : __builtin_amdgcn_make_buffer_rsrc((void*)a.W, 0, (int)a.w_bytes, 0x00020000);
   const int per_split = (total_all + a.nsplit - 1) / a.nsplit;
   const int it_beg = split * per_split;
   const int it_end = it_beg + per_split < total_all ? it_beg + per_split : total_all;
@@ -186,7 +170,22 @@
 #pragma unroll
   for (int i = 0; i < B_INSTR; ++i) {
     const int pc = i * NW + wave;
-    if (w_nk) {
+    if constexpr (WPL) {
+      constexpr int PPP = PLANE_BYTES / 1024;
+      const int pl = pc / PPP, pp = pc % PPP;
+      const unsigned poff = (unsigned)pl * a.wpl_plane_bytes;
+      if (w_nk) {
+        const int r = 16 * pp + (lane >> 2);
+        const int cq = (lane & 3) ^ ((r >> 2) & 3);
+        const int n = n0 + r;
+        voffB[i] = n < a.Cn ? poff + ((unsigned)n * (unsigned)a.Cout_w + (unsigned)cq * 8u) * 2u : OOB;
+      } else {
+        const int k = B_RPP * pp + lane / B_LPR;
+        const int cq = (lane % B_LPR) ^ kstrided_swz<BN>(k);
+        const int n = n0 + cq * 8;
+        voffB[i] = n < a.Cn ? poff + ((unsigned)k * (unsigned)a.Cout_w + (unsigned)n) * 2u : OOB;
+      }
+    } else if (w_nk) {
       const int r = 8 * pc + (lane >> 3);
       const int cq = (lane & 7) ^ ((r >> 1) & 7);
       const int n = n0 + r;
@@ -214,6 +213,23 @@
         boff[j][q] = (unsigned)A_BYTES + (unsigned)r * 128u + (unsigned)(((2 * q + lhi) ^ ((r >> 1) & 7)) * 16);
     } else {
       boff[j][0] = (unsigned)A_BYTES + (unsigned)(4 * lhi) * (unsigned)B_ROWB + (unsigned)(wn * WN + j * 32 + l31) * 4u;
+    }
+  }
+  unsigned poffB[WPL ? TJ : 1][WPL && w_nk ? 4 : 1];
+  if constexpr (WPL) {
+#pragma unroll
+    for (int j = 0; j < TJ; ++j) {
+      if (w_nk) {
+        const int r = wn * WN + j * 32 + l31;
+#pragma unroll
+        for (int c = 0; c < (w_nk ? 4 : 1); ++c)
+          poffB[j][c] = (unsigned)A_BYTES + (unsigned)r * 64u + (unsigned)((c ^ ((r >> 2) & 3)) * 16 + 8 * lhi);
+      } else {
+        const int i16 = lane & 15, g16 = (lane >> 4) & 1;
+        const int k = 4 * lhi + (i16 >> 2);
+        const int colb = (wn * WN + j * 32 + g16 * 16 + (i16 & 3) * 4) * 2;
+        poffB[j][0] = (unsigned)A_BYTES + (unsigned)k * (unsigned)B_ROWB + (unsigned)((((colb >> 4) ^ kstrided_swz<BN>(k)) << 4) | (colb & 15));
+      }
     }
   }
 
@@ -262,11 +278,11 @@
           offA[i] = ok ? (unsigned)(rbase[i] + tapoff) * (unsigned)a.Ck * 4u + cqA[i] : OOB;
           okA[i] = ok;
         }
-        offW = (unsigned)wtap * (unsigned)a.Cin_w * (unsigned)a.Cout_w * 4u;
+        offW = (unsigned)wtap * (unsigned)a.Cin_w * (unsigned)a.Cout_w * (unsigned)W_ESZ;
         tap_dirty = false;
       }
       const unsigned sA = (unsigned)ld_kc * 4u;
-      const unsigned sB = offW + (w_nk ? (unsigned)ld_kc * 4u : (unsigned)ld_kc * (unsigned)a.Cout_w * 4u);
+      const unsigned sB = offW + (w_nk ? (unsigned)ld_kc * (unsigned)W_ESZ : (unsigned)ld_kc * (unsigned)a.Cout_w * (unsigned)W_ESZ);
       if constexpr (xform) {
         constexpr int set = buf;
         const int kch = ld_kc + (int)(cqA[0] >> 2);
diff --git a/mopoe-mimic_amd/csrc/conv_gemm_glds_emu.inc b/mopoe-mimic_amd/csrc/conv_gemm_glds_emu.inc
--- a/mopoe-mimic_amd/csrc/conv_gemm_glds_emu.inc
+++ b/mopoe-mimic_amd/csrc/conv_gemm_glds_emu.inc
@@ -1,10 +1,11 @@
 {
   static_assert(!xform, "EMU: plain operand forms");
   constexpr int NM = 6 * TI * TJ;
-  constexpr int NP = 4 * (TI + TJ);
-  f32x4v ea[2][TI], eb[2][w_nk ? TJ : 1];
-  float ek[2][w_nk ? 1 : TJ][4];
-  Split3 sa[2][TI], sb[2][TJ];
+  constexpr int NP = 4 * (TI + (WPL ? 0 : TJ));
+  f32x4v ea[2][TI], eb[2][w_nk && !WPL ? TJ : 1];
+  float ek[2][w_nk || WPL ? 1 : TJ][4];
+  Split3 sa[2][TI], sb[2][WPL ? 1 : TJ];
+  u32x2 wb[2][WPL ? TJ : 1][3][2];
 
   auto top = [&](int it, auto curc) {
     constexpr int cur = decltype(curc)::value;
@@ -24,7 +25,21 @@
       constexpr int s = decltype(sc)::value, q = 2 * p + s;
 #pragma unroll
       for (int i = 0; i < TI; ++i) lds_frag_f4<0>(ea[s][i], lds_base + stage_off + aoff[i][q]);
-      if constexpr (w_nk) {
+      if constexpr (WPL) {
+        static_for<3>([&](auto plc) {
+          constexpr int pl = decltype(plc)::value;
+#pragma unroll
+          for (int j = 0; j < TJ; ++j) {
+            if constexpr (w_nk) {
+              lds_frag_b64<pl * PLANE_BYTES>(wb[p][WPL ? j : 0][pl][s], lds_base + stage_off + poffB[WPL ? j : 0][w_nk ? 2 * p + s : 0]);
+            } else {
+              s16x4 r;
+              lds_frag_tr64<pl * PLANE_BYTES + (16 * p + 8 * s) * B_ROWB>(r, lds_base + stage_off + poffB[WPL ? j : 0][0]);
+              wb[p][WPL ? j : 0][pl][s] = __builtin_bit_cast(u32x2, r);
+            }
+          }
+        });
+      } else if constexpr (w_nk) {
 #pragma unroll
         for (int j = 0; j < TJ; ++j) lds_frag_f4<0>(eb[s][w_nk ? j : 0], lds_base + stage_off + boff[j][w_nk ? q : 0]);
       } else {
@@ -38,13 +53,21 @@
       }
     });
   };
-  auto fence_e = [&]() {
+  auto fence_e = [&](auto dc) {
+    constexpr int d = decltype(dc)::value;
     MOPOE_DEVICE_ASM("s_waitcnt lgkmcnt(0)" ::: "memory");
+    if constexpr (WPL) {
+#pragma unroll
+      for (int j = 0; j < TJ; ++j)
+#pragma unroll
+        for (int pl = 0; pl < 3; ++pl) { pin_reg(wb[d][WPL ? j : 0][pl][0]); pin_reg(wb[d][WPL ? j : 0][pl][1]); }
+    }
 #pragma unroll
     for (int s = 0; s < 2; ++s) {
 #pragma unroll
       for (int i = 0; i < TI; ++i) pin_reg(ea[s][i]);
-      if constexpr (w_nk) {
+      if constexpr (WPL) {
+      } else if constexpr (w_nk) {
 #pragma unroll
         for (int j = 0; j < TJ; ++j) pin_reg(eb[s][w_nk ? j : 0]);
       } else {
@@ -63,7 +86,7 @@
     if constexpr (f < TI) {
       split3_pair(ea[s][f][e0], ea[s][f][e0 + 1], h, m, l);
       sa[d][f].h[w] = h; sa[d][f].m[w] = m; sa[d][f].l[w] = l;
-    } else {
+    } else if constexpr (!WPL) {
       constexpr int j = f - TI;
       if constexpr (w_nk) split3_pair(eb[s][w_nk ? j : 0][e0], eb[s][w_nk ? j : 0][e0 + 1], h, m, l);
       else split3_pair(ek[s][w_nk ? 0 : j][e0], ek[s][w_nk ? 0 : j][e0 + 1], h, m, l);
@@ -73,7 +96,16 @@
   auto mfma_t = [&](auto tc, auto dc) {
     constexpr int t = decltype(tc)::value, d = decltype(dc)::value;
     constexpr int term = t / (TI * TJ), tile = t % (TI * TJ), i = tile % TI, j = tile / TI;
-    mfma_split_term<term>(acc[i][j], sa[d][i], sb[d][j]);
+    if constexpr (WPL) {
+      const auto& w = wb[d][WPL ? j : 0];
+      Split3 b;
+      b.h = __builtin_shufflevector(w[0][0], w[0][1], 0, 1, 2, 3);
+      b.m = __builtin_shufflevector(w[1][0], w[1][1], 0, 1, 2, 3);
+      b.l = __builtin_shufflevector(w[2][0], w[2][1], 0, 1, 2, 3);
+      mfma_split_term<term>(acc[i][j], sa[d][i], b);
+    } else {
+      mfma_split_term<term>(acc[i][j], sa[d][i], sb[d][WPL ? 0 : j]);
+    }
   };
   using E0 = std::integral_constant<int, 0>; using E1 = std::integral_constant<int, 1>;
   auto all_pieces = [&](auto dc) { static_for<NP>([&](auto uc) { piece(uc, dc); }); };
@@ -81,13 +113,13 @@
   auto chunk2 = [&](int it, auto curc) {
     top(it, curc);
     reads(curc, E0{});
-    fence_e();
+    fence_e(E0{});
     all_pieces(E0{});
     __builtin_amdgcn_sched_barrier(0);
     reads(curc, E1{});
     all_mfma(E0{});
     __builtin_amdgcn_sched_barrier(0);
-    fence_e();
+    fence_e(E1{});
     all_pieces(E1{});
     __builtin_amdgcn_sched_barrier(0);
     all_mfma(E1{});
diff --git a/mopoe-mimic_amd/csrc/gemm_glds_common.inc b/mopoe-mimic_amd/csrc/gemm_glds_common.inc
--- a/mopoe-mimic_amd/csrc/gemm_glds_common.inc
+++ b/mopoe-mimic_amd/csrc/gemm_glds_common.inc
@@ -39,6 +39,24 @@
 #endif
 }
 
+template <int BN>
+__device__ __forceinline__ int kstrided_swz(int k) {
+  static_assert(BN == 64 || BN == 128, "swizzle written for 128- and 256-byte rows");
+  return (BN == 128 ? (k & 3) : ((k >> 1) & 1)) << 2;
+}
+typedef short s16x4 __attribute__((ext_vector_type(4)));
+typedef unsigned int u32x2 __attribute__((ext_vector_type(2)));
+template <int OFF>
+__device__ __forceinline__ void lds_frag_tr64(s16x4& r, unsigned addr) {
+  static_assert(OFF >= 0 && OFF < 65536, "ds offset field");
+  MOPOE_DEVICE_ASM("ds_read_b64_tr_b16 %0, %1 offset:%2" : "=v"(r) : "v"(addr), "n"(OFF) : "memory");
+}
+template <int OFF>
+__device__ __forceinline__ void lds_frag_b64(u32x2& r, unsigned addr) {
+  static_assert(OFF >= 0 && OFF < 65536, "ds offset field");
+  MOPOE_DEVICE_ASM("ds_read_b64 %0, %1 offset:%2" : "=v"(r) : "v"(addr), "n"(OFF) : "memory");
+}
+
 __device__ __forceinline__ void lds_store_b128(unsigned addr, u32x4 v) {
   MOPOE_DEVICE_ASM("ds_write_b128 %0, %1" :: "v"(addr), "v"(v) : "memory");
 }
diff --git a/mopoe-mimic_amd/csrc/split3.inc b/mopoe-mimic_amd/csrc/split3.inc
--- /dev/null
+++ b/mopoe-mimic_amd/csrc/split3.inc
@@ -0,0 +1,25 @@
+#pragma once
+#include "gemm_glds_common.inc"
+
+typedef __bf16 e_bf16x2 __attribute__((ext_vector_type(2)));
+typedef __bf16 e_bf16x8 __attribute__((ext_vector_type(8)));
+typedef float e_f32x2 __attribute__((ext_vector_type(2)));
+struct Split3 { u32x4 h, m, l; };
+
+__device__ __forceinline__ void split3_pair(float a0, float a1, unsigned& h, unsigned& m, unsigned& l) {
+#if defined(MOPOE_DBG_EMU_NOSPLIT)
+  h = __float_as_uint(a0); m = __float_as_uint(a1); l = h;
+  return;
+#endif
+  const e_f32x2 a = {a0, a1};
+  h = __builtin_bit_cast(unsigned, __builtin_convertvector(a, e_bf16x2));
+  float r0 = 0.f, r1 = 0.f, q0 = 0.f, q1 = 0.f;
+  MOPOE_DEVICE_ASM_PURE("v_sub_f32 %0, %1, %2" : "=v"(r0) : "v"(a0), "v"(h << 16));
+  MOPOE_DEVICE_ASM_PURE("v_sub_f32 %0, %1, %2" : "=v"(r1) : "v"(a1), "v"(h & 0xffff0000u));
+  const e_f32x2 r = {r0, r1};
+  m = __builtin_bit_cast(unsigned, __builtin_convertvector(r, e_bf16x2));
+  MOPOE_DEVICE_ASM_PURE("v_sub_f32 %0, %1, %2" : "=v"(q0) : "v"(r0), "v"(m << 16));
+  MOPOE_DEVICE_ASM_PURE("v_sub_f32 %0, %1, %2" : "=v"(q1) : "v"(r1), "v"(m & 0xffff0000u));
+  const e_f32x2 r2 = {q0, q1};
+  l = __builtin_bit_cast(unsigned, __builtin_convertvector(r2, e_bf16x2));
+}
diff --git a/mopoe-mimic_amd/mimic_amd/layout.py b/mopoe-mimic_amd/mimic_amd/layout.py
--- a/mopoe-mimic_amd/mimic_amd/layout.py
+++ b/mopoe-mimic_amd/mimic_amd/layout.py
@@ -113,8 +113,11 @@
             vers = (param_epoch(), [m.weight._version for m in self.mods])
         if force or vers != self.versions:
             with torch.no_grad():
-                torch._foreach_copy_([self.views[id(m)] for m in self.mods], [m.weight.detach() for m in self.mods])
+                self._write()
             self.versions = vers
+
+    def _write(self):
+        torch._foreach_copy_([self.views[id(m)] for m in self.mods], [m.weight.detach() for m in self.mods])
 
     def bind_optimizer(self, on: bool):
         self.synced_by_optimizer = False
@@ -131,6 +134,47 @@
 
     def has(self, mod):
         return id(mod) in self.views or any(m is mod for m in self.mods)
+
+
+class F32Planes(Bf16Weights):
+
+    @staticmethod
+    def eligible(m) -> bool:
+        cin, cout = m.weight.shape[1], m.weight.shape[2]
+        return cin % 4 == 0 and cout % 4 == 0 and min(cin, cout) > 1
+
+    def _active(self):
+        return self.mods[0].weight.is_cuda
+
+    def _build(self):
+        from . import ops
+        dev = self.mods[0].weight.device
+        total = sum(3 * m.weight.numel() for m in self.mods)
+        self.flat = torch.empty(total, dtype=torch.bfloat16, device=dev)
+        off = 0
+        for m in self.mods:
+            n = m.weight.numel()
+            self.views[id(m)] = self.flat[off:off + 3 * n].view(3, n)
+            off += 3 * n
+            ops.bind_wplanes(m.weight, self.views[id(m)])
+        self.versions = None
+
+    def refresh(self, force: bool):
+        if self._active():
+            super().refresh(force)
+
+    def _write(self):
+        from . import ops
+        ops.split_planes([m.weight.detach() for m in self.mods], [self.views[id(m)] for m in self.mods])
+
+    def bind_optimizer(self, on: bool):
+        if not self._active():
+            self.synced_by_optimizer = False
+            return {}
+        return {k: v.view(3, -1) for k, v in super().bind_optimizer(on).items()}
+
+    def get(self, mod):
+        return mod.weight
 
 
 class BnParams(nn.Module):
diff --git a/mopoe-mimic_amd/mimic_amd/nets.py b/mopoe-mimic_amd/mimic_amd/nets.py
--- a/mopoe-mimic_amd/mimic_amd/nets.py
+++ b/mopoe-mimic_amd/mimic_amd/nets.py
@@ -9,7 +9,7 @@
 
 from . import ops
 from .lanes import ModalityLanes
-from .layout import Bf16Weights, BnParams, Indexed, PackedConv, ResBlockParams, param_epoch
+from .layout import Bf16Weights, BnParams, F32Planes, Indexed, PackedConv, ResBlockParams, param_epoch
 from .ops import Geom
 from .trunk import (BackwardArena, BlockSpec, MaskSource, StatsArena, apply_running_updates, stats_needed,
                     trunk_backward, trunk_forward)
@@ -187,6 +187,10 @@
             keep = {id(m) for m in fp32_mods}
             mods = [m for m in self.modules() if isinstance(m, PackedConv) and id(m) not in keep]
             object.__setattr__(self, "_shadow", Bf16Weights(mods))
+        elif ops.F32_WPLANES:
+            mods = [m for m in self.modules() if isinstance(m, PackedConv) and F32Planes.eligible(m)]
+            if mods:
+                object.__setattr__(self, "_shadow", F32Planes(mods))
 
     def _begin_forward(self):
         if self._shadow is not None:
diff --git a/mopoe-mimic_amd/mimic_amd/ops.py b/mopoe-mimic_amd/mimic_amd/ops.py
--- a/mopoe-mimic_amd/mimic_amd/ops.py
+++ b/mopoe-mimic_amd/mimic_amd/ops.py
@@ -2,6 +2,7 @@
 
 import ctypes as C
 import os
+import weakref
 from dataclasses import dataclass
 from functools import lru_cache
 from typing import Optional, Sequence
@@ -10,7 +11,7 @@
 
 _HERE = os.path.dirname(os.path.abspath(__file__))
 LIB_PATH = os.environ.get("MOPOE_HIP_LIB") or os.path.join(os.path.dirname(_HERE), "csrc", "libmopoe_hip.so")
-ABI_VERSION = 20
+ABI_VERSION = 21
 
 RES_A, RES_B = 2.0, 0.3
 BN_EPS = 1e-5
@@ -47,7 +48,11 @@
 
 class _AdamSeg(C.Structure):
     _fields_ = [("p", C.c_void_p), ("g", C.c_void_p), ("m", C.c_void_p), ("v", C.c_void_p), ("p16", C.c_void_p),
-                ("n", C.c_int64)]
+                ("planes", C.c_void_p), ("n", C.c_int64)]
+
+
+class _SplitSeg(C.Structure):
+    _fields_ = [("w", C.c_void_p), ("planes", C.c_void_p), ("n", C.c_int64)]
 
 
 @dataclass(frozen=True)
@@ -208,7 +213,39 @@
 
 
 class _Plan(C.Structure):
-    _fields_ = [("tile", C.c_int32), ("split", C.c_int32)]
+    _fields_ = [("tile", C.c_int32), ("split", C.c_int32), ("wplanes", C.c_void_p)]
+
+
+F32_WPLANES = os.environ.get("MOPOE_F32_WPLANES", "1") != "0"
+WPLANE_TILES = (17, 18, 19)
+_wplanes = {}
+
+
+def bind_wplanes(weight, planes):
+    _wplanes[id(weight)] = (weakref.ref(weight), planes)
+
+
+def unbind_wplanes(weight):
+    _wplanes.pop(id(weight), None)
+
+
+def wplanes_of(weight):
+    e = _wplanes.get(id(weight))
+    if e is None or e[0]() is not weight:
+        return None
+    return e[1]
+
+
+def _with_planes(plan, wp):
+    if plan is None:
+        return None
+    p = plan._obj
+    if p.tile not in WPLANE_TILES:
+        return plan
+    pl = wplanes_of(wp)
+    if pl is None:
+        return plan
+    return C.byref(_Plan(p.tile, p.split, pl.data_ptr()))
 
 
 AUTOTUNE = os.environ.get("MOPOE_AUTOTUNE", "1") not in ("0", "table")
@@ -569,7 +606,7 @@
     key = ("fwd", g, bn_in is not None, mask is not None, out_stats is not None) + (("mix",) if mix is not None else ())
     plan = _tuned_plan(key, lambda: _gather_candidates("fwd", g, nbytes, plain_operand=bn_in is None),
                        lambda ref: launch(ref, _scratch_like(out_stats)))
-    launch(plan, out_stats)
+    launch(_with_planes(plan, wp), out_stats)
     return y
 
 
@@ -612,7 +649,7 @@
     key = ("dgrad", g, relu_bn is not None, bwd_sums is not None)
     plan = _tuned_plan(key, lambda: _gather_candidates("dgrad", g, nbytes, plain_operand=True),
                        lambda ref: launch(ref, _scratch_like(bwd_sums)))
-    launch(plan, bwd_sums)
+    launch(_with_planes(plan, wp), bwd_sums)
     return dx
 
 
@@ -784,17 +821,33 @@
     for i in range(n):
         p_, g_ = params[i], grads[i]
         if g_ is None:
-            arr[i] = _AdamSeg(p_.data_ptr(), None, ms[i].data_ptr(), vs[i].data_ptr(), None, p_.numel())
+            arr[i] = _AdamSeg(p_.data_ptr(), None, ms[i].data_ptr(), vs[i].data_ptr(), None, None, p_.numel())
             continue
         if g_.dtype != torch.float32 or p_.dtype != torch.float32 or g_.numel() != p_.numel():
             raise MopoeHipError("adam_step: parameters and gradients must be fp32 tensors of equal size")
         _dev(p_, g_, ms[i], vs[i])
         lp = lowp[i] if lowp is not None else None
+        planes = lp is not None and lp.dim() == 2 and lp.shape[0] == 3
+        if lp is not None:
+            _dev(lp)
+            if lp.dtype != BF16 or not lp.is_contiguous() or lp.numel() != (3 if planes else 1) * p_.numel():
+                raise MopoeHipError("adam_step: a low-precision copy is a contiguous bf16 tensor of the parameter's size or [3, n] planes")
         arr[i] = _AdamSeg(p_.data_ptr(), g_.data_ptr(), ms[i].data_ptr(), vs[i].data_ptr(),
-                          None if lp is None else lp.data_ptr(), p_.numel())
+                          None if lp is None or planes else lp.data_ptr(), lp.data_ptr() if planes else None, p_.numel())
     lr_dev = lr if isinstance(lr, torch.Tensor) else None
     _check(lib().mopoe_adam_step(arr, n, _p(step) if prep else None, _p(lr_dev), C.c_double(0.0 if lr_dev is not None else float(lr)),
                                  C.c_double(beta1), C.c_double(beta2), C.c_double(eps), _p(coef), _stream()))
+
+
+def split_planes(weights, planes):
+    n = len(weights)
+    arr = (_SplitSeg * n)()
+    for i, (w, pl) in enumerate(zip(weights, planes)):
+        _dev(w, pl)
+        if w.dtype != torch.float32 or not w.is_contiguous() or pl.dtype != BF16 or not pl.is_contiguous() or pl.numel() != 3 * w.numel():
+            raise MopoeHipError("split_planes: an fp32 weight and [3, n] bf16 planes")
+        arr[i] = _SplitSeg(w.data_ptr(), pl.data_ptr(), w.numel())
+    _check(lib().mopoe_split_planes(arr, n, _stream()))
 
 
 def colsum(x, out=None):
```
